# sdiehl/sonic

Measured on AMD Instinct MI355X. Metric: prove() proofs/sec, higher is better.
Workload: dtype u32 limbs (Fq 12x32, Fr 8x32 Montgomery); 1 GPU; prove(): rndCircuit n=2^18, Q=2, SRS d=2^21 (d=8n >= 7n, Protocol.hs:54); n=262144, Q=2, d=2097152, process_group=none (plain single-process run), legs=headline only (the other legs: --full)

## Files before the change

sonic_amd/csrc/device.hip:

```cpp
#include <stdarg.h>
#include <string.h>
#include <memory>
#include <string>
#include <vector>
#include "internal.hpp"

namespace sonic {

static thread_local char g_err[512] = "";
void set_error(const char* fmt, ...) {
  va_list ap;
  va_start(ap, fmt);
  vsnprintf(g_err, sizeof g_err, fmt, ap);
  va_end(ap);
}

Profiler& profiler() { static Profiler p; return p; }
void Profiler::collect() {
  std::lock_guard<std::mutex> g(mu);
  for (auto& kv : recs) {
    auto& tot = totals[kv.first];
    for (auto& r : kv.second) {
      hipEventSynchronize(r.b);
      float ms = 0;
      hipEventElapsedTime(&ms, r.a, r.b);
      tot.first += ms; tot.second += 1;
      hipEventDestroy(r.a); hipEventDestroy(r.b);
    }
    kv.second.clear();
  }
}
void Profiler::reset() { collect(); std::lock_guard<std::mutex> g(mu); totals.clear(); }

static std::mutex g_init_mu;
static int g_device = -1;
static int g_device_count = -1;
static std::vector<DeviceCtx*> g_ctx;
static thread_local DeviceCtx* t_ctx = nullptr;

static int device_count_locked() {
  if (g_device_count >= 0) return g_device_count;
  setenv("GPU_MAX_HW_QUEUES", "8", 0);
  int n = 0;
  hipError_t e = hipGetDeviceCount(&n);
  if (e != hipSuccess || n <= 0) {
    (void)hipGetLastError();
    set_error("no HIP device available (%s): libsonic_hip has no CPU fallback", e == hipSuccess ? "0 devices" : hipGetErrorString(e));
    throw HipFail{SONIC_ERR_NO_DEVICE};
  }
  g_device_count = n;
  g_ctx.assign((size_t)n, nullptr);
  return n;
}
static DeviceCtx* ctx_locked(int dev) {
  if (!g_ctx[(size_t)dev]) {
    std::unique_ptr<DeviceCtx> c(new DeviceCtx());
    c->dev = dev;
    HIP_OK(hipStreamCreateWithFlags(&c->stream, hipStreamNonBlocking));
    g_ctx[(size_t)dev] = c.release();
  }
  return g_ctx[(size_t)dev];
}
int default_device_ordinal() { std::lock_guard<std::mutex> g(g_init_mu); return g_device; }
void unlink_one_shot_of(const sonic_srs* s) {
  std::lock_guard<std::mutex> g(g_init_mu);
  for (DeviceCtx* c : g_ctx) {
    if (!c) continue;
    std::lock_guard<std::mutex> g2(c->one_shot_mu);
    for (size_t i = 0; i < c->one_shot.size();) {
      if (static_cast<OneShotShell*>(c->one_shot[i])->srs == s) c->one_shot.erase(c->one_shot.begin() + (long)i);
      else i++;
    }
  }
}

DeviceScope::DeviceScope(int dev) : ctx_(nullptr), prev_ctx_(t_ctx), prev_dev_(-1) {
  if (t_ctx && (dev < 0 || t_ctx->dev == dev)) { ctx_ = t_ctx; return; }
  std::lock_guard<std::mutex> g(g_init_mu);
  const int n = device_count_locked();
  if (dev < 0) {
    if (g_device < 0) {
      const char* lr = getenv("LOCAL_RANK");
      g_device = lr ? atoi(lr) % n : 0;
      if (g_device < 0) g_device = 0;
    }
    dev = g_device;
  }
  if (dev >= n) { set_error("device %d out of range (%d device%s)", dev, n, n == 1 ? "" : "s"); throw HipFail{SONIC_ERR_INVALID_ARG}; }
  if (hipGetDevice(&prev_dev_) != hipSuccess) { (void)hipGetLastError(); prev_dev_ = -1; }
  if (prev_dev_ != dev) HIP_OK(hipSetDevice(dev));
  try { ctx_ = ctx_locked(dev); } catch (...) { if (prev_dev_ >= 0 && prev_dev_ != dev) (void)hipSetDevice(prev_dev_); throw; }
  t_ctx = ctx_;
}
DeviceScope::~DeviceScope() {
  if (ctx_ == prev_ctx_) return;
  t_ctx = prev_ctx_;
  if (prev_dev_ >= 0 && prev_dev_ != ctx_->dev) (void)hipSetDevice(prev_dev_);
}
const NttTables& device_ntt_tables(int log2n) {
  DeviceCtx& c = current_ctx();
  std::lock_guard<std::mutex> g(c.pool_mu);
  NttTables*& t = c.prover_ntt[log2n];
  if (!t) {
    std::unique_ptr<NttTables> nt(new NttTables());
    hipStream_t st = nullptr;
    HIP_OK(hipStreamCreateWithFlags(&st, hipStreamNonBlocking));
    try { nt->ensure(st, log2n); HIP_OK(hipStreamSynchronize(st)); } catch (...) { (void)hipStreamDestroy(st); throw; }
    (void)hipStreamDestroy(st);
    t = nt.release();
  }
  return *t;
}
DeviceCtx& current_ctx() {
  if (!t_ctx) { set_error("internal: no device scope on this thread"); throw HipFail{SONIC_ERR_HIP}; }
  return *t_ctx;
}

CallLease::CallLease() : c_(nullptr), owner_(&current_ctx()) {
  {
    std::lock_guard<std::mutex> g(owner_->pool_mu);
    if (!owner_->pool.empty()) { c_ = owner_->pool.back(); owner_->pool.pop_back(); }
  }
  if (!c_) {
    std::unique_ptr<CallCtx> c(new CallCtx());
    HIP_OK(hipStreamCreateWithFlags(&c->st, hipStreamNonBlocking));
    c_ = c.release();
  }
}
CallLease::~CallLease() {
  (void)hipStreamSynchronize(c_->st);
  std::lock_guard<std::mutex> g(owner_->pool_mu);
  owner_->pool.push_back(c_);
}

}

using namespace sonic;

extern "C" {

int sonic_init(int device_ordinal) {
  API_HOST_BEGIN
  {
    std::lock_guard<std::mutex> g(g_init_mu);
    const int n = device_count_locked();
    if (device_ordinal >= n) { set_error("device %d out of range (%d device%s)", device_ordinal, n, n == 1 ? "" : "s"); return SONIC_ERR_INVALID_ARG; }
    if (g_device < 0 && device_ordinal >= 0) g_device = device_ordinal;
  }
  int dev;
  { DeviceScope scope(-1); dev = scope.ctx().dev; }
  HIP_OK(hipSetDevice(dev));
  API_END
}

int sonic_device_count(int* out) {
  if (!out) return SONIC_ERR_INVALID_ARG;
  try { std::lock_guard<std::mutex> g(g_init_mu); *out = device_count_locked(); } catch (const HipFail& f) { *out = 0; return f.code; }
  return SONIC_OK;
}

int sonic_hip_versions(int* build, int* runtime) {
  if (build) *build = HIP_VERSION;
  if (runtime) { int v = 0; if (hipRuntimeGetVersion(&v) != hipSuccess) v = 0; *runtime = v; }
  return SONIC_OK;
}

int sonic_last_error(char* buf, size_t cap) {
  if (!buf || cap == 0) return SONIC_ERR_INVALID_ARG;
  strncpy(buf, g_err, cap - 1);
  buf[cap - 1] = 0;
  return SONIC_OK;
}

int sonic_device_sync(void) { API_BEGIN HIP_OK(hipStreamSynchronize(default_stream())); HIP_OK(hipDeviceSynchronize()); API_END }

int sonic_abi_version(void) { return SONIC_ABI_VERSION; }

static int device_of_pointer(const void* p) {
  hipPointerAttribute_t a;
  if (p && hipPointerGetAttributes(&a, p) == hipSuccess) return a.device;
  (void)hipGetLastError();
  return -1;
}
int sonic_dev_alloc(size_t bytes, void** out) { return sonic_dev_alloc_on(-1, bytes, out); }
int sonic_dev_alloc_on(int device, size_t bytes, void** out) { API_BEGIN_ON(device) if (!out) return SONIC_ERR_INVALID_ARG; HIP_OK(hipMalloc(out, bytes ? bytes : 16)); API_END }
int sonic_dev_free(void* p) { API_BEGIN_ON(device_of_pointer(p)) HIP_OK(hipFree(p)); API_END }
int sonic_dev_upload(void* dst, const void* src, size_t bytes) { API_BEGIN_ON(device_of_pointer(dst)) HIP_OK(hipMemcpy(dst, src, bytes, hipMemcpyHostToDevice)); API_END }
int sonic_dev_download(void* dst, const void* src, size_t bytes) { API_BEGIN_ON(device_of_pointer(src)) HIP_OK(hipMemcpy(dst, src, bytes, hipMemcpyDeviceToHost)); API_END }

int sonic_profile_enable(int on) { profiler().on = on != 0; return SONIC_OK; }
int sonic_profile_reset(void) { profiler().reset(); return SONIC_OK; }
int sonic_profile_get(const char* kernel, double* total_ms, int64_t* launches) {
  if (!kernel) return SONIC_ERR_INVALID_ARG;
  profiler().collect();
  std::lock_guard<std::mutex> g(profiler().mu);
  auto it = profiler().totals.find(kernel);
  if (total_ms) *total_ms = it == profiler().totals.end() ? 0.0 : it->second.first;
  if (launches) *launches = it == profiler().totals.end() ? 0 : it->second.second;
  return SONIC_OK;
}
int sonic_profile_names(char* buf, size_t cap) {
  if (!buf || cap == 0) return SONIC_ERR_INVALID_ARG;
  profiler().collect();
  std::lock_guard<std::mutex> g(profiler().mu);
  std::string s;
  for (auto& kv : profiler().totals) { s += kv.first; s += "\n"; }
  strncpy(buf, s.c_str(), cap - 1);
  buf[cap - 1] = 0;
  return SONIC_OK;
}

}
```

sonic_amd/csrc/internal.hpp:

```cpp
#pragma once
#include <atomic>
#include <exception>
#include "common.hpp"
#include "g1.hpp"
#include "msm.hpp"

struct sonic_srs;
struct sonic_prover;

namespace sonic {

struct NttTables;

struct CallCtx;
struct DeviceCtx {
  int dev = -1;
  hipStream_t stream = nullptr;
  std::mutex call_mu;
  std::mutex pool_mu;
  std::vector<CallCtx*> pool;
  std::vector<void*> lanes;
  NttTables* ntt = nullptr;
  DevBuf mul_a, mul_b, mul_flags;
  std::atomic<int> sort_staged{-1};
  std::atomic<int> ntt_big{-1};
  std::map<int, NttTables*> prover_ntt;
  std::mutex one_shot_mu;
  std::vector<void*> one_shot;
};
const NttTables& device_ntt_tables(int log2n);
void drop_one_shot_of(const sonic_srs* s);
struct OneShotShell { const sonic_srs* srs; sonic_prover* p; };
void unlink_one_shot_of(const sonic_srs* s);
class DeviceScope {
 public:
  explicit DeviceScope(int dev = -1);
  ~DeviceScope();
  DeviceScope(const DeviceScope&) = delete;
  DeviceScope& operator=(const DeviceScope&) = delete;
  DeviceCtx& ctx() const { return *ctx_; }
 private:
  DeviceCtx* ctx_;
  DeviceCtx* prev_ctx_;
  int prev_dev_;
};
DeviceCtx& current_ctx();
int default_device_ordinal();
inline hipStream_t default_stream() { return current_ctx().stream; }
inline std::mutex& call_mutex() { return current_ctx().call_mu; }
struct CallCtx { hipStream_t st = nullptr; MsmWorkspace ws; };
class CallLease {
 public:
  CallLease();
  ~CallLease();
  CallLease(const CallLease&) = delete;
  CallLease& operator=(const CallLease&) = delete;
  hipStream_t st() const { return c_->st; }
  MsmWorkspace& ws() const { return c_->ws; }
 private:
  CallCtx* c_;
  DeviceCtx* owner_;
};

#define API_BEGIN_ON(dev) try { ::sonic::DeviceScope _scope(dev);
#define API_BEGIN API_BEGIN_ON(-1)
#define API_HOST_BEGIN try {
#define API_CATCH                                                               \
  } catch (const ::sonic::HipFail& f) { return f.code; }                        \
  catch (const std::exception& e) { ::sonic::set_error("%s", e.what()); return SONIC_ERR_HIP; }
#define API_END API_CATCH return SONIC_OK;

int64_t srs_d(const sonic_srs* s);
int srs_cached_id(const sonic_srs* s, int (*make)(const sonic_srs*, uint8_t*), uint8_t out[32]);

void fr_to_mont_enqueue(hipStream_t st, Fr* d, long n, int* d_err);
void fr_from_mont_enqueue(hipStream_t st, Fr* d, long n);
void fr_check_enqueue(hipStream_t st, const Fr* d, long n, int* d_err);
void points_from_bytes_enqueue(hipStream_t st, const uint8_t* d_in96, PointArrayMut out, long n, int* d_err, long inf_ok);
void points_subgroup_check_enqueue(hipStream_t st, PointArray in, long n, int* d_err);
void points_to_bytes_enqueue(hipStream_t st, PointArray in, uint8_t* d_out96, long n);
int read_flags(hipStream_t st, DevBuf& flags);
void msm_blocking(hipStream_t st, MsmWorkspace& ws, const MsmPlan& pl, PointArray d_pts, const Fr* d_sc, long n, bool mont,
                  uint8_t* out96, uint8_t* out_partial192);
struct G2Affine;
void srs_generate_g2(hipStream_t st, long d, const Fr& x_std, const Fr& alpha_std, G2Affine* h0, G2Affine* h1);
void g2_points_to_bytes_enqueue(hipStream_t st, const G2Affine* in, uint8_t* d_out, long n);
void g2_points_from_bytes_enqueue(hipStream_t st, const uint8_t* d_in, G2Affine* out, long n, int* d_err);

void g1_decompress_enqueue(hipStream_t st, const uint8_t* d_in48, PointArrayMut out, uint8_t* d_bytes96, uint8_t* d_flags, long n, bool check_subgroup);
void g2_decompress_enqueue(hipStream_t st, const uint8_t* d_in96, G2Affine* out, uint8_t* d_bytes192, uint8_t* d_flags, long n, bool check_subgroup);
void g1_compress_enqueue(hipStream_t st, PointArray in, uint8_t* d_out48, long n);
void g2_compress_enqueue(hipStream_t st, const G2Affine* in, uint8_t* d_out96, long n);
void g1_validate_enqueue(hipStream_t st, const uint8_t* d_in96, G1Affine* out, uint8_t* d_flags, long n);

struct NttTables {
  int log2n = 0;
  DevBuf fwd, inv;
  DevBuf ninv;
  void ensure(hipStream_t st, int log2n);
};
void ntt_forward_enqueue(hipStream_t st, const NttTables& tw, Fr* d, int log2n);
void ntt_inverse_enqueue(hipStream_t st, const NttTables& tw, Fr* d, int log2n);
void ntt_inverse_of_product_enqueue(hipStream_t st, const NttTables& tw, Fr* d, const Fr* other, int log2n);
void fr_pointwise_mul_enqueue(hipStream_t st, Fr* a, const Fr* b, long n);
void fr_scale_enqueue(hipStream_t st, Fr* a, long n, const Fr* d_s);
void fr_bitrev_permute_enqueue(hipStream_t st, Fr* d, int log2n);

void poly_scale_powers_enqueue(hipStream_t st, const Fr* in, Fr* out, long n, long e0, const Fr* d_x, const Fr* d_xinv);
void poly_prefix_sum_enqueue(hipStream_t st, Fr* d, long n, DevBuf& tmp);
void poly_quotient_enqueue(hipStream_t st, const Fr* prefix, Fr* q, long n, long lo, const Fr* d_z, const Fr* d_zinv);

}
```

sonic_amd/csrc/prove.hip:

```cpp
#include "prover.hpp"
#include "witness_tree.hpp"

namespace sonic {

constexpr long PROVE_TWO_LEVEL_MAX_TERMS = 1L << 21;
static bool prove_two_level(const MsmPlan& pl, int k, bool last, long nmax) {
  if (last || k <= 1 || pl.NB < (1 << 18)) return false;
  const char* e = getenv("SONIC_PROVE_TWO_LEVEL");
  if (e && (e[0] == '0' || e[0] == '1') && !e[1]) return e[0] == '1';
  return nmax <= PROVE_TWO_LEVEL_MAX_TERMS;
}
static int prove_segment(const MsmPlan& pl, int k, bool last, bool two_level) {
  const bool big = pl.NB >= (1 << 18);
  if (last) return big ? 16 : 4;
  if (k <= 1) return big ? 8 : 4;
  if (!big) return 16;
  const char* e = getenv("SONIC_PROVE_SEGMENT");
  const int v = e ? atoi(e) : 0;
  return v >= 8 && v <= 1024 ? v : (two_level ? 32 : 64);
}

MsmJob commit_job(hipStream_t st, const sonic_srs* srs, const Fr* poly, long lo, long len, long maxm, MsmSlot* slot, int* d_flags) {
  const long d = srs->d, shift = d - maxm;
  long i0 = -d - shift - lo, i1 = d - shift - lo + 1;
  if (i0 < 0) i0 = 0;
  if (i1 > len) i1 = len;
  if (i1 < i0) i1 = i0;
  flag_nonzero_enqueue(st, poly, i0, d_flags, FLAG_SRS_INDEX);
  flag_nonzero_enqueue(st, poly + i1, len - i1, d_flags, FLAG_SRS_INDEX);
  const long ih = -shift - lo;
  if (ih >= i0 && ih < i1) flag_nonzero_enqueue(st, poly + ih, 1, d_flags, FLAG_SRS_INDEX);
  return MsmJob{srs->basis(1) + (lo + i0 + shift + d), poly + i0, i1 - i0, slot};
}

void run_jobs(hipStream_t st, const sonic_srs* srs, MsmWorkspace& ws, const MsmJob* jobs, int k, bool last, bool exposed) {
  if (k <= 0) return;
  long nmax = 0;
  for (int j = 0; j < k; j++) nmax = std::max(nmax, jobs[j].n);
  MsmPlan pl = srs_msm_plan(srs, nmax);
  const bool tree = last || exposed || pl.NB <= (1 << 17);
  if (k > 1 && msm_can_batch(pl)) {
    pl.two_level = prove_two_level(pl, k, last, nmax);
    msm_plan_set_segment(pl, prove_segment(pl, k, last, pl.two_level));
    pl.tree = tree;
    msm_enqueue_batch(st, ws, pl, jobs, k, true);
    return;
  }
  for (int j = 0; j < k; j++) {
    MsmPlan p1 = srs_msm_plan(srs, jobs[j].n);
    msm_plan_set_segment(p1, prove_segment(p1, 1, false, false));
    p1.tree = tree;
    msm_enqueue_batch(st, ws, p1, &jobs[j], 1, true);
  }
}

static void eval_prefix_enqueue(hipStream_t st, Scratch& sc, const Fr* poly, long lo, long len, const Fr* zpair, Fr* d_fz) {
  sc.reserve(len);
  sc.scan.ensure(sizeof(Fr) * (len / 1024 + 2));
  poly_scale_powers_enqueue(st, poly, sc.D.as<Fr>(), len, lo, zpair, zpair + 1);
  poly_prefix_sum_enqueue(st, sc.D.as<Fr>(), len, sc.scan);
  HIP_OK(hipMemcpyAsync(d_fz, sc.D.as<Fr>() + (len - 1), sizeof(Fr), hipMemcpyDeviceToDevice, st));
}

static MsmJob quotient_job(hipStream_t st, const sonic_srs* srs, const Fr* q, long lo, long len, MsmSlot* slot, int* d_flags) {
  const long d = srs->d, qn = len - 1;
  long i0 = -d - lo, i1 = d - lo + 1;
  if (i0 < 0) i0 = 0;
  if (i1 > qn) i1 = qn;
  if (i1 < i0) i1 = i0;
  flag_nonzero_enqueue(st, q, i0, d_flags, FLAG_SRS_INDEX);
  flag_nonzero_enqueue(st, q + i1, qn - i1, d_flags, FLAG_SRS_INDEX);
  return MsmJob{srs->basis(0) + (lo + i0 + d), q + i0, i1 - i0, slot};
}

MsmJob open_job(hipStream_t st, const sonic_srs* srs, Scratch& sc, const Fr* poly, long lo, long len,
                       const Fr* zpair, Fr* d_fz, MsmSlot* slot, int* d_flags) {
  sc.reserve(len);
  eval_prefix_enqueue(st, sc, poly, lo, len, zpair, d_fz ? d_fz : sc.fz_discard.as<Fr>());
  poly_quotient_enqueue(st, sc.D.as<Fr>(), sc.q.as<Fr>(), len, lo, zpair, zpair + 1);
  return quotient_job(st, srs, sc.q.as<Fr>(), lo, len, slot, d_flags);
}

MsmJob open_job_at_zero(hipStream_t st, const sonic_srs* srs, const Fr* poly, long len, Fr* d_fz, MsmSlot* slot, int* d_flags) {
  const long d = srs->d;
  HIP_OK(hipMemcpyAsync(d_fz, poly, sizeof(Fr), hipMemcpyDeviceToDevice, st));
  const long qn = len - 1;
  long i1 = d + 1;
  if (i1 > qn) i1 = qn;
  flag_nonzero_enqueue(st, poly + 1 + i1, qn - i1, d_flags, FLAG_SRS_INDEX);
  return MsmJob{srs->basis(0) + d, poly + 1, i1, slot};
}

struct PendingOpen { const Fr* poly; long lo, len; const Fr* zp; Fr* fz; MsmSlot* slot; long slot_index; Scratch* sc; };
static void open_batch_set(OpenBatch& b, int i, Scratch& sc, const Fr* poly, long len, const Fr* zp, Fr* fz) {
  sc.reserve(len);
  sc.scan.ensure(sizeof(Fr) * (len / 1024 + 2));
  b.poly[i] = poly; b.D[i] = sc.D.as<Fr>(); b.q[i] = sc.q.as<Fr>(); b.tiles[i] = sc.scan.as<Fr>();
  b.zpair[i] = zp; b.fz[i] = fz ? fz : sc.fz_discard.as<Fr>();
}
static void open_jobs_batched(hipStream_t st, const sonic_srs* srs, const PendingOpen* ops, int k, int* d_flags, MsmJob* jobs_out) {
  for (int at = 0; at < k;) {
    int e = at;
    OpenBatch b;
    memset(&b, 0, sizeof b);
    while (e < k && e - at < OPEN_BATCH_MAX && ops[e].lo == ops[at].lo && ops[e].len == ops[at].len) {
      open_batch_set(b, e - at, *ops[e].sc, ops[e].poly, ops[e].len, ops[e].zp, ops[e].fz);
      e++;
    }
    b.k = e - at;
    const long lo = ops[at].lo, len = ops[at].len;
    open_batch_enqueue(st, b, lo, len);
    for (int i = at; i < e; i++) jobs_out[i] = quotient_job(st, srs, ops[i].sc->q.as<Fr>(), lo, len, ops[i].slot, d_flags);
    at = e;
  }
}

bool bytes_are_zero(const uint8_t* p, size_t n) { for (size_t i = 0; i < n; i++) if (p[i]) return false; return true; }

}

int upload_fr_mont(hipStream_t st, DevBuf& dst, const uint8_t* src, long count, int* d_flags) {
  dst.ensure(sizeof(Fr) * (count > 0 ? count : 1));
  if (count > 0) {
    HIP_OK(hipMemcpyAsync(dst.p, src, 32 * count, hipMemcpyHostToDevice, st));
    fr_to_mont_enqueue(st, dst.as<Fr>(), count, d_flags);
  }
  return 0;
}

int flags_to_status(int f, const char* who) {
  if (f & FLAG_BAD_ENCODING) { set_error("%s: non-canonical field element in input", who); return SONIC_ERR_BAD_ENCODING; }
  if (f & FLAG_SRS_INDEX) { set_error("%s: a non-zero coefficient needs an SRS element outside [-d, d] or the omitted g^alpha (index -1)", who); return SONIC_ERR_SRS_INDEX; }
  return SONIC_OK;
}

void prover_hand_over(sonic_prover_t* p, const CircuitView& c) {
  p->circuit_has_runs = circuit_runs_hint(c, RUN_TILE);
  p->pend.view = c;
  if (c.csr) csr_layout(c, p->pend.layout);
  p->pend.set = true;
}

static void upload_i32(hipStream_t st, DevBuf& dst, const std::vector<int32_t>& src) {
  dst.ensure(sizeof(int32_t) * (src.empty() ? 1 : src.size()));
  if (!src.empty()) HIP_OK(hipMemcpyAsync(dst.p, src.data(), sizeof(int32_t) * src.size(), hipMemcpyHostToDevice, st));
}
static void prover_upload_circuit(sonic_prover_t* p, hipStream_t st, int* d_flags) {
  const CircuitView& c = p->pend.view;
  const long n = p->n, Q = p->Q;
  if (c.csr) {
    const CsrLayout& L = p->pend.layout;
    sonic_prover::CsrBufs& b = p->sp;
    upload_i32(st, b.row_ptr, L.row_ptr); upload_i32(st, b.col, L.col);
    upload_i32(st, b.col_ptr, L.col_ptr); upload_i32(st, b.row, L.row);
    upload_i32(st, b.chunk_row, L.chunk_row); upload_i32(st, b.chunk_begin, L.chunk_begin); upload_i32(st, b.row_chunk, L.row_chunk);
    upload_fr_mont(st, b.val, c.val, L.nnz, d_flags);
    upload_fr_mont(st, b.cval, L.cval.data(), L.nnz, d_flags);
    b.nnz = L.nnz;
    b.nchunks = (long)L.chunk_row.size();
    b.partial.ensure(sizeof(Fr) * (b.nchunks > 0 ? b.nchunks : 1));
    b.h_row_ptr = L.row_ptr;
  } else {
    upload_fr_mont(st, p->wL, c.wL, Q * n, d_flags);
    upload_fr_mont(st, p->wR, c.wR, Q * n, d_flags);
    upload_fr_mont(st, p->wO, c.wO, Q * n, d_flags);
  }
  upload_fr_mont(st, p->cs, c.cs, Q, d_flags);
  p->csr = c.csr;
  p->pend.set = false;
}

static int prover_load_circuit(sonic_prover* p, const CircuitView& c) {
  hipStream_t st = p->st;
  prover_hand_over(p, c);
  HIP_OK(hipMemsetAsync(p->flags.p, 0, 4, st));
  prover_upload_circuit(p, st, p->flags.as<int>());
  int f = read_flags(st, p->flags);
  p->pend = sonic_prover::PendingCircuit();
  if (f) return flags_to_status(f, c.csr ? "sonic_prover_new_csr" : "sonic_prover_new");
  return SONIC_OK;
}

static void s_of_y_of(sonic_prover* p, hipStream_t st, const Fr* ypow, Fr* out) {
  if (p->csr) s_of_y_csc_enqueue(st, p->sp.col_ptr.as<int32_t>(), p->sp.row.as<int32_t>(), p->sp.cval.as<Fr>(), ypow, p->n, p->Q, out);
  else s_of_y_enqueue(st, p->wL.as<Fr>(), p->wR.as<Fr>(), p->wO.as<Fr>(), ypow, p->n, p->Q, out);
}
static void s_of_u_of(sonic_prover* p, hipStream_t st, const Fr* upow, Fr* out) {
  sonic_prover::CsrBufs& b = p->sp;
  if (p->csr) s_of_u_csr_enqueue(st, b.row_ptr.as<int32_t>(), b.col.as<int32_t>(), b.val.as<Fr>(), b.chunk_row.as<int32_t>(), b.chunk_begin.as<int32_t>(),
                                 b.nchunks, b.row_chunk.as<int32_t>(), upow, p->n, p->Q, out, b.partial.as<Fr>());
  else s_of_u_enqueue(st, p->wL.as<Fr>(), p->wR.as<Fr>(), p->wO.as<Fr>(), upow, p->n, p->Q, out, p->tmp);
}

extern "C" {

size_t sonic_proof_size(int64_t Q) { return ProofLayout{Q}.proof_bytes(); }

static int prover_new_entry(const char* who, const sonic_srs_t* srs, const CircuitView& c, sonic_prover_t** out) {
  API_BEGIN_ON(srs_device(srs))
  if (!srs || !c.cs || !out) { set_error("%s: bad argument (need n >= 1, Q >= 1)", who); return SONIC_ERR_INVALID_ARG; }
  int rc = prover_admits(who, srs, c);
  if (rc) return rc;
  return prover_new_impl(srs, c, out);
  API_END
}
int sonic_prover_new(const sonic_srs_t* srs, int64_t n, int64_t Q, const uint8_t* wL, const uint8_t* wR, const uint8_t* wO,
                     const uint8_t* cs, sonic_prover_t** out) {
  return prover_new_entry("sonic_prover_new", srs, dense_view(n, Q, wL, wR, wO, cs), out);
}
int sonic_prover_new_csr(const sonic_srs_t* srs, int64_t n, int64_t Q, const int64_t* row_ptr, const int64_t* col, const uint8_t* val,
                         const uint8_t* cs, sonic_prover_t** out) {
  return prover_new_entry("sonic_prover_new_csr", srs, csr_view(n, Q, row_ptr, col, val, cs), out);
}

}

int prover_admits(const char* who, const sonic_srs* srs, const CircuitView& c) {
  if (circuit_args_ok(c) && srs->d < 7 * c.n) {
    set_error("Parameter d is not large enough: %ld should be greater than %ld", (long)srs->d, (long)(7 * c.n));
    return SONIC_ERR_D_TOO_SMALL;
  }
  return circuit_validate(who, c);
}

int prover_new_impl(const sonic_srs_t* srs, const CircuitView& c, sonic_prover_t** out) {
  const long n = c.n, Q = c.Q;
  const ProofLayout L{Q};
  for (long q = 0; c.csr && q < Q; q++) {
    Fr k; memcpy(k.l, c.cs + 32 * q, 32);
    if (!fp_is_canonical(k)) { set_error("sonic_prover_new_csr: non-canonical constant cs[%ld]", q); return SONIC_ERR_BAD_ENCODING; }
  }
  std::unique_ptr<sonic_prover> p(new sonic_prover());
  p->srs = srs; p->n = n; p->Q = Q;
  p->device = srs_device(srs);
  {
    const MsmPlan probe = srs_msm_plan(srs, 3 * n);
    p->small_plan = msm_can_batch(probe) && probe.NB <= (1 << 17);
  }
  auto mkstream = [](hipStream_t* s) { HIP_OK(hipStreamCreateWithFlags(s, hipStreamNonBlocking)); };
  mkstream(&p->st);
  mkstream(&p->ts);
  hipStream_t st = p->st;
  p->flags.alloc(8);
  int rc_c = prover_load_circuit(p.get(), c);
  if (rc_c) return rc_c;
  const long tlen = 7 * n + 9;
  int lg = 0;
  while ((1L << lg) < tlen) lg++;
  p->log2m = lg;
  p->ntt = &device_ntt_tables(lg);
  const long M = 1L << lg;
  p->fa.alloc(sizeof(Fr) * M); p->fb.alloc(sizeof(Fr) * M);
  p->r1.alloc(sizeof(Fr) * (3 * n + 5));
  p->sy0.alloc(sizeof(Fr) * (3 * n + 1));
  p->syj.resize(Q);
  for (auto& b : p->syj) b.alloc(sizeof(Fr) * (3 * n + 1));
  p->su.alloc(sizeof(Fr) * (2 * n + Q + 1));
  p->pw.alloc(sizeof(Fr) * (3 * n + Q + 2));
  p->kpow.alloc(sizeof(Fr) * Q);
  p->S.alloc(sizeof(Fr) * L.transcript_len()); p->PAIRS.alloc(sizeof(Fr) * 2 * L.n_pairs());
  p->slots.alloc(sizeof(MsmSlot) * L.slots_total());
  p->use_graph = getenv("SONIC_PROVE_GRAPH") && atoi(getenv("SONIC_PROVE_GRAPH")) != 0;
  HIP_OK(hipHostMalloc((void**)&p->h_tr, 32 * L.transcript_len(), hipHostMallocDefault));
  HIP_OK(hipHostMalloc((void**)&p->h_pairs, sizeof(Fr) * 2 * L.n_pairs(), hipHostMallocDefault));
  HIP_OK(hipHostMalloc((void**)&p->h_slots, sizeof(MsmSlot) * L.slots_total(), hipHostMallocDefault));
  HIP_OK(hipHostMalloc((void**)&p->h_fr, 32 * L.F(), hipHostMallocDefault));
  HIP_OK(hipHostMalloc((void**)&p->h_flags, 8, hipHostMallocDefault));
  HIP_OK(hipHostMalloc((void**)&p->h_root, 32, hipHostMallocDefault));
  p->h_flags[0] = p->h_flags[1] = 0;
  p->frout.alloc(sizeof(Fr) * L.F());
  p->frstd.alloc(sizeof(Fr) * L.F());
  HIP_OK(hipMemsetAsync(p->frout.p, 0, sizeof(Fr) * L.F(), st));
  HIP_OK(hipMemsetAsync(p->slots.p, 0, sizeof(MsmSlot) * L.slots_total(), st));
  memset(p->h_slots, 0, sizeof(MsmSlot) * L.slots_total());
  auto mkev = [](hipEvent_t* e) { HIP_OK(hipEventCreateWithFlags(e, hipEventDisableTiming)); };
  mkev(&p->ev_r1); mkev(&p->ev_sy0); mkev(&p->ev_t); mkev(&p->ev_su);
  p->ev_syj.resize(Q, nullptr);
  for (auto& e : p->ev_syj) mkev(&e);
  if (p->small_plan) {
    const char* le = getenv("SONIC_FUSED_LANES");
    p->n_lanes = std::min(std::max(le ? atoi(le) : N_LANES, 1), N_LANES);
  }
  for (int i = 0; i < p->n_lanes; i++) {
    Lane& l = p->lanes[i];
    mkstream(&l.st);
    mkev(&l.done);
    mkev(&l.prep);
  }
  if (p->small_plan) {
    for (int c = 0; c < (L.K() > MSM_MAX_JOBS ? 2 : 1); c++) {
      mkstream(&p->chain[c].st);
      mkev(&p->chain[c].done);
    }
  }
  HIP_OK(hipStreamSynchronize(st));
  *out = p.release();
  return SONIC_OK;
}

extern "C" {

int sonic_prover_set_assignment(sonic_prover_t* p, const uint8_t* aL, const uint8_t* aR, const uint8_t* aO) {
  API_BEGIN_ON(p ? p->device : -1)
  if (!p || !aL || !aR || !aO) return SONIC_ERR_INVALID_ARG;
  std::lock_guard<std::mutex> g(p->mu);
  if (p->in_flight) { set_error("sonic_prover_set_assignment: a submitted proof is still reading the current assignment (collect it first)"); return SONIC_ERR_INVALID_ARG; }
  hipStream_t st = p->st;
  HIP_OK(hipMemsetAsync(p->flags.p, 0, 4, st));
  upload_fr_mont(st, p->aL, aL, p->n, p->flags.as<int>());
  upload_fr_mont(st, p->aR, aR, p->n, p->flags.as<int>());
  upload_fr_mont(st, p->aO, aO, p->n, p->flags.as<int>());
  int f = read_flags(st, p->flags);
  if (f) {
    p->have_assignment = false;
    return flags_to_status(f, "sonic_prover_set_assignment");
  }
  p->have_assignment = true;
  p->assignment_changed();
  API_END
}

}

struct GroupQueue {
  sonic_prover_t* const p;
  const sonic_srs* const srs;
  const ProofLayout L;
  int* const flags; MsmSlot* const slots; Fr* const frout;
  const SlotShare* const sh;
  Lane* cur = nullptr;
  std::vector<PendingOpen> pend;
  std::vector<std::function<void()>> after_flush;
  std::vector<std::function<void()>> deferred_small;
  enum Side { BESIDE_GROUP, BEHIND_CHAIN };

  explicit GroupQueue(sonic_prover_t* p_)
      : p(p_), srs(p_->srs), L{p_->Q}, flags(p_->flags.as<int>()), slots(p_->slots.as<MsmSlot>()), frout(p_->frout.as<Fr>()),
        sh(p_->share_world > 1 ? p_->share.row(p_->share_rank) : nullptr) {
    p->next_lane = 0;
    p->slot_ran.assign((size_t)L.slots_total(), 0);
    p->fr_valid.assign((size_t)L.F(), 0);
  }
  bool on(int ph) const { return ((p->phases >> ph) & 1u) != 0; }
  bool own(long slot) const { return !sh || sh[slot].hi > sh[slot].lo; }
  bool first_piece(long slot) const { return !sh || (sh[slot].hi > sh[slot].lo && sh[slot].lo == 0); }
  void push(MsmJob job, long slot) {
    if (sh) {
      long t0, t1;
      share_term_range(sh[slot], job.n, &t0, &t1);
      job.points = job.points + t0; job.scalars += t0; job.n = t1 - t0;
      if (job.n <= 0) return;
    }
    p->slot_ran[(size_t)slot] = 1;
    cur->jobs[cur->njobs++] = job;
  }
  void issue_opens() {
    if (pend.empty()) return;
    MsmJob oj[MSM_MAX_JOBS];
    open_jobs_batched(cur->st, srs, pend.data(), (int)pend.size(), flags, oj);
    for (size_t i = 0; i < pend.size(); i++) push(oj[i], pend[i].slot_index);
    pend.clear();
  }
  void flush(bool last = false) {
    if (!cur) return;
    issue_opens();
    if (p->fused) p->fused_jobs.insert(p->fused_jobs.end(), cur->jobs, cur->jobs + cur->njobs);
    else run_jobs(cur->st, srs, cur->ws, cur->jobs, cur->njobs, last, p->share_world >= 4);
    cur->njobs = 0;
    if (p->fused) deferred_small.insert(deferred_small.end(), after_flush.begin(), after_flush.end());
    else for (auto& f : after_flush) f();
    after_flush.clear();
  }
  void begin_group(hipEvent_t e) {
    flush();
    cur = &p->pick(e);
    cur->njobs = 0;
  }
  void begin_t_group(Lane& lane_t) {
    if (on(PH_T)) HIP_OK(hipStreamWaitEvent(lane_t.st, p->ev_t, 0));
    cur = &lane_t; cur->njobs = 0;
  }
  void make_room() { if (cur->njobs + (int)pend.size() == MSM_MAX_JOBS) flush(); }
  void commit(int ph, const Fr* poly, long lo, long len, long maxm, long slot) {
    if (!on(ph) || !own(slot)) return;
    make_room();
    push(commit_job(cur->st, srs, poly, lo, len, maxm, &slots[slot], flags), slot);
  }
  void commit_runs(int ph, const Fr* poly, long lo, long len, long maxm, long j) {
    const long slot = L.S(j), Q = L.Q;
    if (!on(ph) || !own(slot)) return;
    make_room();
    MsmJob job = commit_job(cur->st, srs, poly, lo, len, maxm, &slots[slot], flags);
    const long ntiles = job.n / RUN_TILE;
    if (ntiles > 0) {
      if ((long)p->runs.size() < Q) p->runs.resize((size_t)Q);
      sonic_prover::RunBufs& rb = p->runs[(size_t)j];
      if (!rb.masked_ev) HIP_OK(hipEventCreateWithFlags(&rb.masked_ev, hipEventDisableTiming));
      rb.masked.ensure(sizeof(Fr) * job.n); rb.val.ensure(sizeof(Fr) * ntiles); rb.uniform.ensure(4 * ntiles);
      rb.scal.ensure(sizeof(Fr) * 2 * ntiles); rb.pts.ensure(sizeof(G1Affine) * 2 * ntiles);
      run_tiles_enqueue(cur->st, job.scalars, job.n, rb.masked.as<Fr>(), rb.val.as<Fr>(), rb.uniform.as<uint32_t>());
      HIP_OK(hipEventRecord(rb.masked_ev, cur->st));
      const long first = (long)((job.points.p - srs->basis(1).p) / (long)job.points.stride);
      sonic_prover::RunBufs* rbp = &rb;
      side([this, rbp, first, ntiles, j] {
        hipStream_t ms = p->st;
        HIP_OK(hipStreamWaitEvent(ms, rbp->masked_ev, 0));
        run_terms_enqueue(ms, rbp->val.as<Fr>(), rbp->uniform.as<uint32_t>(), ntiles, srs->prefix() + first, first, rbp->scal.as<Fr>(), rbp->pts.as<G1Affine>());
        msm_enqueue(ms, p->runs_ws, msm_plan(2 * ntiles), PointArray::packed(rbp->pts.as<G1Affine>()), rbp->scal.as<Fr>(), 2 * ntiles, true, &slots[L.S_extra(j)]);
      }, BEHIND_CHAIN);
      job.scalars = rb.masked.as<Fr>();
      p->slot_ran[(size_t)L.S_extra(j)] = 1;
    }
    push(job, slot);
  }
  void commit_sym(int ph, const Fr* su, long lo, long len, long n) {
    if (!on(ph) || !own(L.C())) return;
    const long d = srs->d;
    make_room();
    MsmJob job = commit_job(cur->st, srs, su, lo, len, d, &slots[L.C()], flags);
    job.points = srs->sym() + 1; job.scalars = su + (n + 1); job.n = n; job.table_stride = d + 1;
    push(job, L.C());
    p->slot_ran[(size_t)L.C_extra()] = 1;
    side([this, su, d, n] { msm_enqueue(p->st, p->runs_ws, msm_plan(L.Q), srs->basis(1) + (d + n + 1), su + (2 * n + 1), L.Q, true, &slots[L.C_extra()]); }, BEHIND_CHAIN);
  }
  void open(int ph, const Fr* poly, long lo, long len, const Fr* zp, long fr, long slot) {
    if (!on(ph) || !own(slot)) return;
    make_room();
    Scratch& sc = p->fused ? p->fused_scratch() : cur->sc[cur->njobs + (int)pend.size()];
    pend.push_back(PendingOpen{poly, lo, len, zp, fr >= 0 ? &frout[fr] : nullptr, &slots[slot], slot, &sc});
    if (fr >= 0 && first_piece(slot)) p->fr_valid[(size_t)fr] = 1;
  }
  void side(std::function<void()> fn, Side when) {
    if (when == BEHIND_CHAIN ? !p->fused : cur->njobs == 0) fn();
    else (when == BEHIND_CHAIN ? deferred_small : after_flush).push_back(std::move(fn));
  }
  void run_chains() {
    if (!p->fused || p->fused_jobs.empty()) return;
    for (int i = 0; i < p->n_lanes; i++) HIP_OK(hipEventRecord(p->lanes[i].prep, p->lanes[i].st));
    const int total = (int)p->fused_jobs.size();
    const int nchunks = (total + MSM_MAX_JOBS - 1) / MSM_MAX_JOBS, per = (total + nchunks - 1) / nchunks;
    for (int c = 0, at = 0; c < nchunks; c++, at += per) {
      Lane& cl = p->chain[c & 1];
      if (c < 2) for (int i = 0; i < p->n_lanes; i++) HIP_OK(hipStreamWaitEvent(cl.st, p->lanes[i].prep, 0));
      const int k = std::min(per, total - at);
      const MsmJob* jobs = &p->fused_jobs[(size_t)at];
      long nmax = 0;
      for (int j = 0; j < k; j++) nmax = std::max(nmax, jobs[j].n);
      MsmPlan pl = srs_msm_plan(srs, nmax);
      pl.tree = true;
      pl.accum_block = 128;
      msm_enqueue_batch(cl.st, cl.ws, pl, jobs, k, true);
    }
    p->fused_jobs.clear();
  }
  void drain_deferred() {
    for (auto& f : deferred_small) f();
    deferred_small.clear();
  }
  void join() {
    hipStream_t ms = p->st;
    for (int i = 0; i < p->n_lanes; i++) { Lane& l = p->lanes[i]; HIP_OK(hipEventRecord(l.done, l.st)); HIP_OK(hipStreamWaitEvent(ms, l.done, 0)); }
    if (p->fused) for (auto& l : p->chain) if (l.st) { HIP_OK(hipEventRecord(l.done, l.st)); HIP_OK(hipStreamWaitEvent(ms, l.done, 0)); }
  }
};

struct ProofPass {
  const long n, Q, d;
  const long r_lo, r_len, s_lo, s_len, t_lo, t_len, u_lo, u_len;
  const Fr* const PR;
  bool need_g0, need_T, need_su, need_j_any = false;
  std::vector<uint8_t> need_j;
  long last_j = -1;
  int last_group;
  bool g0_queued = false;
  const Fr* pair(long i) const { return PR + 2 * i; }
  ProofPass(sonic_prover_t* p, const GroupQueue& q)
      : n(p->n), Q(p->Q), d(p->srs->d), r_lo(-2 * n - 4), r_len(3 * n + 5), s_lo(-n), s_len(3 * n + 1), t_lo(-4 * n - 8), t_len(7 * n + 9),
        u_lo(-n), u_len(2 * n + Q + 1), PR(p->PAIRS.as<Fr>()), need_j((size_t)Q, 0) {
    const ProofLayout& L = q.L;
    need_su = q.own(L.C()) || q.own(L.Qv());
    for (long j = 0; j < Q; j++) {
      need_j[(size_t)j] = q.own(L.S(j)) || q.own(L.W(j)) || q.own(L.Wp(j));
      need_j_any = need_j_any || need_j[(size_t)j];
      if (need_j[(size_t)j]) last_j = j;
      need_su = need_su || q.own(L.Qj(j));
    }
    need_g0 = q.own(L.R) || q.own(L.Wa) || q.own(L.Wb);
    need_T = q.own(L.T) || q.own(L.Wt);
    last_group = need_T ? 3 : need_su ? 2 : need_j_any ? 1 : 0;
  }
};

static void enqueue_group0(sonic_prover_t* p, GroupQueue& q, ProofPass& w) {
  if (!w.need_g0 || w.g0_queued) return;
  w.g0_queued = true;
  const ProofLayout& L = q.L;
  const Fr* r1 = p->r1.as<Fr>();
  q.begin_group(p->ev_r1);
  q.commit(PH_R, r1, w.r_lo, w.r_len, w.n, L.R);
  q.open(PH_OPEN, r1, w.r_lo, w.r_len, w.pair(L.pZ), L.a, L.Wa);
  q.open(PH_OPEN, r1, w.r_lo, w.r_len, w.pair(L.pYZ), L.b, L.Wb);
  q.flush(w.last_group == 0);
}

static void enqueue_polynomials(sonic_prover_t* p, GroupQueue& q, ProofPass& w) {
  const ProofLayout& L = q.L;
  const long n = w.n, Q = w.Q;
  hipStream_t ms = p->st;
  int* flags = q.flags;
  Fr *r1 = p->r1.as<Fr>(), *sy = p->sy0.as<Fr>(), *pw = p->pw.as<Fr>(), *fa = p->fa.as<Fr>(), *fb = p->fb.as<Fr>();
  auto ready = [&](hipEvent_t e) { HIP_OK(hipEventRecord(e, ms)); };
  if (p->pend_asg[0]) {
    upload_fr_mont(ms, p->aL, p->pend_asg[0], n, flags + 1);
    upload_fr_mont(ms, p->aR, p->pend_asg[1], n, flags + 1);
    upload_fr_mont(ms, p->aO, p->pend_asg[2], n, flags + 1);
    p->pend_asg[0] = nullptr;
    p->assignment_changed();
  }
  if (p->pend_wit.set) {
    for (DevBuf* a : {&p->aL, &p->aR, &p->aO}) a->ensure(sizeof(Fr) * (size_t)n);
    if (p->pend_wit.ready) HIP_OK(hipStreamWaitEvent(ms, p->pend_wit.ready, 0));
    witness_load_enqueue(p, ms, p->pend_wit.v, 1, p->aL.as<Fr>(), p->aR.as<Fr>(), p->aO.as<Fr>(), n, flags + 1);
    p->pend_wit.set = false;
    p->assignment_changed();
  }
  if (p->pend_cs) {
    upload_fr_mont(ms, p->cs, p->pend_cs, Q, flags + 1);
    p->pend_cs = nullptr;
  }
  if ((w.need_g0 || w.need_T) && q.on(PH_R)) build_r1_enqueue(ms, p->aL.as<Fr>(), p->aR.as<Fr>(), p->aO.as<Fr>(), p->S.as<Fr>(), n, r1);
  ready(p->ev_r1);
  if (p->pend.set) {
    enqueue_group0(p, q, w);
    prover_upload_circuit(p, ms, flags + 1);
  }
  if (w.need_T && q.on(PH_T)) {
    poly_scale_powers_enqueue(ms, nullptr, pw, 2 * n + Q + 1, -n, w.pair(L.pY), w.pair(L.pY) + 1);
    s_of_y_of(p, ms, pw, sy);
    HIP_OK(hipMemcpyAsync(p->kpow.p, pw + (2 * n + 1), sizeof(Fr) * Q, hipMemcpyDeviceToDevice, ms));
  }
  ready(p->ev_sy0);
  if (w.need_T && q.on(PH_T)) {
    hipStream_t ts = p->ts;
    const long M = 1L << p->log2m;
    HIP_OK(hipStreamWaitEvent(ts, p->ev_sy0, 0));
    t_operands_enqueue(ts, r1, w.r_len, w.r_lo, sy, w.s_lo - w.r_lo, w.s_len, w.pair(L.pY), fa, fb, M);
    ntt_forward_enqueue(ts, *p->ntt, fa, p->log2m);
    ntt_forward_enqueue(ts, *p->ntt, fb, p->log2m);
    ntt_inverse_of_product_enqueue(ts, *p->ntt, fa, fb, p->log2m);
    sub_k_of_y_enqueue(ts, fa + (0 - w.t_lo), p->cs.as<Fr>(), p->kpow.as<Fr>(), Q, flags, 0);
    HIP_OK(hipEventRecord(p->ev_t, ts));
  }
  for (long j = 0; j < Q; j++) {
    if (w.need_j[(size_t)j] && q.on(PH_HSCS)) {
      poly_scale_powers_enqueue(ms, nullptr, pw, 2 * n + Q + 1, -n, w.pair(L.pYj(j)), w.pair(L.pYj(j)) + 1);
      if (!p->prepared || q.own(L.W(j)) || q.own(L.Wp(j))) s_of_y_of(p, ms, pw, p->syj[j].as<Fr>());
      if (p->prepared && q.own(L.S(j))) s_diag_part_enqueue(ms, pw, n, Q, p->diag[j].as<Fr>(), p->yq[j].as<Fr>());
    }
    ready(p->ev_syj[j]);
  }
  if (w.need_su && q.on(PH_HSCW)) {
    poly_scale_powers_enqueue(ms, nullptr, pw, 3 * n + 1, -n, w.pair(L.pU), w.pair(L.pU) + 1);
    s_of_u_of(p, ms, pw, p->su.as<Fr>());
  }
  ready(p->ev_su);
}

static void enqueue_t_group(sonic_prover_t* p, GroupQueue& q, const ProofPass& w, Lane& lane_t) {
  const ProofLayout& L = q.L;
  const Fr* t = p->fa.as<Fr>();
  q.begin_t_group(lane_t);
  q.commit(PH_T, t, w.t_lo, w.t_len, w.d, L.T);
  q.open(PH_OPEN, t, w.t_lo, w.t_len, w.pair(L.pZ), -1, L.Wt);
  q.flush(true);
}

static void enqueue_groups(sonic_prover_t* p, GroupQueue& q, ProofPass& w) {
  const ProofLayout& L = q.L;
  const long n = w.n, Q = w.Q, d = w.d;
  MsmSlot* slots = q.slots;
  Fr* su = p->su.as<Fr>();
  Lane& lane_t = p->t_lane(p->ev_sy0);
  if (q.on(PH_OPEN) && q.first_piece(L.Wt)) {
    OpenBatch eb;
    memset(&eb, 0, sizeof eb);
    eb.k = 1;
    open_batch_set(eb, 0, lane_t.sc[MSM_MAX_JOBS - 1], p->sy0.as<Fr>(), w.s_len, w.pair(L.pZ), &q.frout[L.s]);
    open_batch_enqueue(lane_t.st, eb, w.s_lo, w.s_len, false);
    p->fr_valid[(size_t)L.s] = 1;
  }
  enqueue_group0(p, q, w);
  for (long j = 0; j < Q; j++) {
    if (!w.need_j[(size_t)j]) continue;
    Fr* syj = p->syj[j].as<Fr>();
    q.begin_group(p->ev_syj[j]);
    if (p->prepared) q.commit(PH_HSCS, p->diag[j].as<Fr>(), n + 1, n, d, L.S(j));
    else if (p->runs_on) q.commit_runs(PH_HSCS, syj, w.s_lo, w.s_len, d, j);
    else q.commit(PH_HSCS, syj, w.s_lo, w.s_len, d, L.S(j));
    q.open(PH_HSCS, syj, w.s_lo, w.s_len, w.pair(L.pZj(j)), L.s_j(j), L.W(j));
    q.open(PH_HSCW, syj, w.s_lo, w.s_len, w.pair(L.pU), -1, L.Wp(j));
    q.flush(w.last_group == 1 && j == w.last_j);
    if (p->prepared && q.on(PH_HSCS) && q.first_piece(L.S(j))) {
      Lane* ln = q.cur;
      p->slot_ran[(size_t)L.S_extra(j)] = 1;
      q.side([p, ln, j, Q, out = &slots[L.S_extra(j)]] {
        msm_enqueue(ln->st, ln->ws, p->cq_tab.p ? msm_plan_tables(Q, CQ_TAB_C, CQ_TAB_W, Q) : msm_plan(Q),
                    PointArray::packed(p->cq_tab.p ? p->cq_tab.as<G1Affine>() : p->cq.as<G1Affine>()), p->yq[j].as<Fr>(), Q, true, out);
      }, GroupQueue::BESIDE_GROUP);
    }
  }
  if (w.need_su) {
    q.begin_group(p->ev_su);
    if (p->sym_on) q.commit_sym(PH_HSCW, su, w.u_lo, w.u_len, n);
    else q.commit(PH_HSCW, su, w.u_lo, w.u_len, d, L.C());
    for (long j = 0; j < Q; j++) q.open(PH_HSCW, su, w.u_lo, w.u_len, w.pair(L.pYj(j)), L.sp_j(j), L.Qj(j));
    q.open(PH_QV, su, w.u_lo, w.u_len, w.pair(L.pV), -1, L.Qv());
  }
  q.flush(w.last_group == 2 && q.sh != nullptr);
  if (w.need_T) enqueue_t_group(p, q, w, lane_t);
  q.run_chains();
  q.drain_deferred();
}

static void enqueue_proof(sonic_prover_t* p) {
  const ProofLayout L{p->Q};
  hipStream_t st = p->st;
  int* flags = p->flags.as<int>();
  HIP_OK(hipMemsetAsync(flags, 0, 8, st));
  Fr* S = p->S.as<Fr>();
  HIP_OK(hipMemcpyAsync(S, p->h_tr, 32 * L.transcript_len(), hipMemcpyHostToDevice, st));
  fr_to_mont_enqueue(st, S, L.transcript_len(), flags);
  HIP_OK(hipMemcpyAsync(p->PAIRS.p, p->h_pairs, sizeof(Fr) * 2 * L.n_pairs(), hipMemcpyHostToDevice, st));
  GroupQueue q(p);
  ProofPass w(p, q);
  enqueue_polynomials(p, q, w);
  enqueue_groups(p, q, w);
  q.join();
  Fr* frstd = p->frstd.as<Fr>();
  HIP_OK(hipMemcpyAsync(frstd, q.frout, sizeof(Fr) * L.F(), hipMemcpyDeviceToDevice, st));
  fr_from_mont_enqueue(st, frstd, L.F());
  const long KS = p->sym_on ? L.slots_total() : (p->prepared || p->runs_on) ? L.C_extra() : L.K();
  HIP_OK(hipMemcpyAsync(p->h_slots, q.slots, sizeof(MsmSlot) * KS, hipMemcpyDeviceToHost, st));
  HIP_OK(hipMemcpyAsync(p->h_fr, frstd, 32 * L.F(), hipMemcpyDeviceToHost, st));
  HIP_OK(hipMemcpyAsync(p->h_flags, flags, 8, hipMemcpyDeviceToHost, st));
}

static void decide_modes(sonic_prover_t* p) {
  {
    const char* re = getenv("SONIC_PROVE_RUNS");
    const int mode = re ? atoi(re) : -1;
    const bool size_ok = mode == 1 ? 3 * p->n + 1 >= 8 * RUN_TILE : p->n >= (1L << 16);
    p->runs_on = mode != 0 && size_ok && (mode == 1 || p->circuit_has_runs) && !p->prepared && p->share_world <= 1 && p->srs->prefix().p != nullptr;
  }
  {
    const char* se = getenv("SONIC_PROVE_SYM");
    const int mode = se ? atoi(se) : -1;
    p->sym_on = mode != 0 && (mode == 1 || p->n >= (1L << 17)) && p->share_world <= 1 && p->srs->sym().p != nullptr;
  }
  {
    const MsmPlan probe = srs_msm_plan(p->srs, 3 * p->n);
    const char* fe = getenv("SONIC_PROVE_FUSED");
    const int mode = fe ? atoi(fe) : -1;
    p->fused = mode != 0 && p->small_plan && msm_can_batch(probe) && p->share_world <= 1;
    p->fused_jobs.clear();
    p->fused_sc_next = 0;
  }
}

static void share_replan_if_needed(sonic_prover_t* p) {
  if (p->share_world <= 1 || (p->share_planned && p->share_planned_prepared == p->prepared)) return;
  const long n = p->n, Q = p->Q;
  const MsmPlan mp = srs_msm_plan(p->srs, 3 * n);
  const ShareCosts costs = ShareCosts::from_env();
  p->share = share_plan(n, Q, p->prepared, p->share_world, mp.NB, mp.W, costs);
  uint64_t h = 1469598103934665603ull;
  auto mix = [&](uint64_t v) { for (int i = 0; i < 8; i++) { h ^= (v >> (8 * i)) & 0xff; h *= 1099511628211ull; } };
  auto mixd = [&](double d) { uint64_t v; memcpy(&v, &d, 8); mix(v); };
  mix((uint64_t)n); mix((uint64_t)Q); mix(p->prepared ? 1 : 0); mix((uint64_t)p->share_world); mix((uint64_t)mp.NB); mix((uint64_t)mp.W);
  mixd(costs.per_job_buckets); mixd(costs.r1); mixd(costs.sy); mixd(costs.su); mixd(costs.tprod);
  p->share_plan_tag = (int32_t)(uint32_t)(h ^ (h >> 32));
  p->share_planned = true; p->share_planned_prepared = p->prepared;
}

static void challenge_pairs_host(sonic_prover_t* p, const uint8_t* transcript) {
  const ProofLayout L{p->Q};
  const long np = L.n_pairs();
  std::vector<Fr> v((size_t)np), pre((size_t)np);
  auto tr = [&](long k) { Fr a; memcpy(a.l, transcript + 32 * k, 32); return fp_to_mont(a); };
  v[L.pY] = tr(L.y); v[L.pZ] = tr(L.z); v[L.pYZ] = fp_mul(v[L.pY], v[L.pZ]); v[L.pU] = tr(L.u()); v[L.pV] = tr(L.v());
  for (long j = 0; j < L.Q; j++) { v[L.pYj(j)] = tr(L.y_j(j)); v[L.pZj(j)] = tr(L.z_j(j)); }
  Fr acc = Fr::one();
  for (long i = 0; i < np; i++) { pre[i] = acc; acc = fp_mul(acc, v[i].is_zero() ? Fr::one() : v[i]); }
  Fr inv = fp_inv(acc);
  for (long i = np - 1; i >= 0; i--) {
    p->h_pairs[2 * i] = v[i];
    if (v[i].is_zero()) { p->h_pairs[2 * i + 1] = v[i]; continue; }
    p->h_pairs[2 * i + 1] = fp_mul(inv, pre[i]);
    inv = fp_mul(inv, v[i]);
  }
}

static int prove_enqueue(sonic_prover_t* p, const uint8_t* transcript) {
  API_BEGIN_ON(p->device)
  p->t_begin = std::chrono::steady_clock::now();
  const ProofLayout L{p->Q};
  hipStream_t st = p->st;
  for (long k = L.n_blinders; k < L.transcript_len(); k++)
    if (bytes_are_zero(transcript + 32 * k, 32)) { set_error("prove: transcript element %ld is zero: Laurent evaluation at 0 divides by zero", k); return SONIC_ERR_INEXACT_DIVISION; }
  if (p->share_world > 1 && p->phases != PH_ALL) { set_error("prove: a shared proof runs with a caller-supplied transcript only"); return SONIC_ERR_INVALID_ARG; }
  decide_modes(p);
  share_replan_if_needed(p);
  memcpy(p->h_tr, transcript, 32 * L.transcript_len());
  challenge_pairs_host(p, transcript);
  const bool pending = p->pend.set || p->pend_asg[0] != nullptr || p->pend_wit.set || p->pend_cs != nullptr;
  const bool want_graph = p->use_graph && p->proofs_done >= 1 && !profiler().on && p->phases == PH_ALL && !pending;
  const bool replay = want_graph && p->graph != nullptr;
  const bool capturing = want_graph && !replay && !p->graph_tried;
  struct CaptureGuard {
    hipStream_t st; bool active = false;
    ~CaptureGuard() { if (active) { hipGraph_t g = nullptr; (void)hipStreamEndCapture(st, &g); if (g) (void)hipGraphDestroy(g); } }
  } capture{st};
  if (capturing) { p->graph_tried = true; HIP_OK(hipStreamBeginCapture(st, hipStreamCaptureModeRelaxed)); capture.active = true; }
  if (!replay) enqueue_proof(p);
  if (capturing) {
    hipGraph_t g = nullptr;
    capture.active = false;
    HIP_OK(hipStreamEndCapture(st, &g));
    hipError_t ge = hipGraphInstantiate(&p->graph, g, nullptr, nullptr, 0);
    (void)hipGraphDestroy(g);
    if (ge != hipSuccess) { p->graph = nullptr; set_error("prove: hipGraphInstantiate failed: %s", hipGetErrorString(ge)); return SONIC_ERR_HIP; }
  }
  if (replay || capturing) HIP_OK(hipGraphLaunch(p->graph, st));
  p->t_enq = std::chrono::steady_clock::now();
  API_END
}

namespace {
struct ShareHeader { uint32_t magic, version; int32_t rank, world; int64_t Q; int32_t flags, plan_tag; };
constexpr uint32_t SHARE_VERSION = 2;
constexpr uint32_t SHARE_MAGIC = 0x48534e53u;
G1XYZZ g1_sum(const G1XYZZ& a, const G1XYZZ& b) { return g1_add(a, b); }
}
extern "C" size_t sonic_proof_share_size(int64_t Q) {
  const size_t K = (size_t)ProofLayout{Q}.K(), F = (size_t)ProofLayout{Q}.F();
  return sizeof(ShareHeader) + K * 8 + K * 192 + F * 32 + F * 4;
}

static bool await_proof(sonic_prover_t* p, bool share) {
  HIP_OK(hipStreamSynchronize(p->st));
  p->proofs_done++;
  if (!getenv("SONIC_DEBUG_TIMING")) return false;
  char who[32] = "prove";
  if (share) snprintf(who, sizeof who, "share %d/%d", p->share_rank, p->share_world);
  fprintf(stderr, "[sonic] %s: enqueue %.3f ms, then waited %.3f ms for the device\n", who,
          std::chrono::duration<double, std::milli>(p->t_enq - p->t_begin).count(),
          std::chrono::duration<double, std::milli>(std::chrono::steady_clock::now() - p->t_enq).count());
  return true;
}

static int prove_finish_share(sonic_prover_t* p, uint8_t* out_share) {
  API_BEGIN_ON(p->device)
  const long Q = p->Q;
  const ProofLayout L{Q};
  const int K = (int)L.K(), F = (int)L.F();
  await_proof(p, true);
  const MsmSlot* hs = p->h_slots;
  memset(out_share, 0, sonic_proof_share_size(Q));
  ShareHeader h{SHARE_MAGIC, SHARE_VERSION, p->share_rank, p->share_world > 1 ? p->share_world : 1, Q, *p->h_flags, p->share_world > 1 ? p->share_plan_tag : 0};
  memcpy(out_share, &h, sizeof h);
  uint8_t* o = out_share + sizeof h;
  for (int i = 0; i < K; i++) {
    SlotShare s; s.lo = 0; s.hi = SHARE_ONE;
    if (p->share_world > 1) s = p->share.row(p->share_rank)[i];
    memcpy(o, &s.lo, 4); memcpy(o + 4, &s.hi, 4); o += 8;
  }
  std::vector<G1XYZZ> sums((size_t)L.slots_total());
  for (long i = 0; i < L.slots_total(); i++) sums[(size_t)i] = p->slot_ran[(size_t)i] ? msm_finish_host(hs[i]) : G1XYZZ::inf();
  fold_side_slots(L, p->prepared || p->runs_on, p->sym_on, sums.data(), sums.data() + K, g1_sum);
  memcpy(o, sums.data(), 192 * (size_t)K);
  o += 192 * (size_t)K;
  for (int i = 0; i < F; i++, o += 32) if (p->fr_valid[(size_t)i]) memcpy(o, p->h_fr + 32 * i, 32);
  for (int i = 0; i < F; i++, o += 4) { const int32_t v = p->fr_valid[(size_t)i]; memcpy(o, &v, 4); }
  API_END
}

extern "C" int sonic_proof_from_shares(int64_t Q, int world, const uint8_t* shares, const uint8_t* transcript, uint8_t* out_proof) {
  try {
  if (Q < 1 || world < 1 || !shares || !transcript || !out_proof) return SONIC_ERR_INVALID_ARG;
  const int K = (int)ProofLayout{Q}.K(), F = (int)ProofLayout{Q}.F();
  const size_t sz = sonic_proof_share_size(Q);
  std::vector<const uint8_t*> by_rank((size_t)world, nullptr);
  int flags = 0;
  int32_t tag0 = 0;
  for (int r = 0; r < world; r++) {
    ShareHeader h;
    memcpy(&h, shares + sz * r, sizeof h);
    if (r == 0) tag0 = h.plan_tag;
    if (h.magic == SHARE_MAGIC && h.version == SHARE_VERSION && h.plan_tag != tag0) {
      set_error("sonic_proof_from_shares: the ranks planned the proof with different parameters (share %d: tag %08x, share 0: %08x) -- their SRS handles "
                "run different MSM plans (window tables built on one GPU and not on another?) or their SONIC_SHARE_COST_* environments differ", r, (unsigned)h.plan_tag, (unsigned)tag0);
      return SONIC_ERR_INVALID_ARG;
    }
    if (h.magic != SHARE_MAGIC || h.version != SHARE_VERSION || h.Q != Q || h.world != world || h.rank < 0 || h.rank >= world || by_rank[(size_t)h.rank]) {
      set_error("sonic_proof_from_shares: share %d is not one of %d distinct shares of a Q = %ld proof", r, world, (long)Q); return SONIC_ERR_INVALID_ARG; }
    by_rank[(size_t)h.rank] = shares + sz * r;
    flags |= h.flags;
  }
  if (flags) return flags_to_status(flags, "prove");
  std::vector<G1XYZZ> sums((size_t)K, G1XYZZ::inf());
  for (int i = 0; i < K; i++) {
    std::vector<std::pair<uint32_t, uint32_t>> pieces;
    for (int r = 0; r < world; r++) {
      const uint8_t* b = by_rank[(size_t)r] + sizeof(ShareHeader);
      uint32_t lo, hi;
      memcpy(&lo, b + 8 * i, 4); memcpy(&hi, b + 8 * i + 4, 4);
      if (hi <= lo) continue;
      pieces.push_back({lo, hi});
      G1XYZZ part;
      memcpy(&part, b + 8 * K + 192 * (size_t)i, 192);
      sums[(size_t)i] = g1_add(sums[(size_t)i], part);
    }
    std::sort(pieces.begin(), pieces.end());
    uint32_t at = 0;
    for (auto& pc : pieces) { if (pc.first != at) break; at = pc.second; }
    if (at != SHARE_ONE) { set_error("sonic_proof_from_shares: the pieces of MSM %d do not cover its terms exactly once", i); return SONIC_ERR_INVALID_ARG; }
  }
  std::vector<uint8_t> pts(96 * (size_t)K), frs(32 * (size_t)F);
  g1_canonical_bytes_host_batch(sums.data(), K, pts.data());
  for (int i = 0; i < F; i++) {
    bool got = false;
    for (int r = 0; r < world && !got; r++) {
      const uint8_t* b = by_rank[(size_t)r] + sizeof(ShareHeader) + 8 * (size_t)K + 192 * (size_t)K;
      int32_t v; memcpy(&v, b + 32 * (size_t)F + 4 * (size_t)i, 4);
      if (v) { memcpy(&frs[32 * (size_t)i], b + 32 * (size_t)i, 32); got = true; }
    }
    if (!got) { set_error("sonic_proof_from_shares: no share reports evaluation %d", i); return SONIC_ERR_INVALID_ARG; }
  }
  proof_layout(Q, pts.data(), frs.data(), transcript, out_proof);
  } catch (const std::exception& e) { set_error("%s", e.what()); return SONIC_ERR_HIP; }
  return SONIC_OK;
}

static bool slots_folded(const MsmSlot* hs, long K) {
  for (long i = 0; i < K; i++) if (hs[i].W > 1 && hs[i].pad1 == 0) return false;
  return true;
}
static void finish_slots_host(const MsmSlot* hs, long K, G1XYZZ* out, int max_threads) {
  long two_level = 0;
  for (long i = 0; i < K; i++) two_level += hs[i].pad1 == 3;
  const int nt = !slots_folded(hs, K) ? (int)std::min<long>(K, max_threads) : (two_level >= 8 ? std::min(4, max_threads) : 1);
  ThreadGroup th;
  for (int w = 1; w < nt; w++) th.emplace_back([=] { for (long i = w; i < K; i += nt) out[i] = msm_finish_host(hs[i]); });
  for (long i = 0; i < K; i += nt) out[i] = msm_finish_host(hs[i]);
}

static int prove_finish(sonic_prover_t* p, uint8_t* out_proof) {
  API_BEGIN_ON(p->device)
  const long Q = p->Q;
  const ProofLayout L{Q};
  const int K = (int)L.K();
  const uint8_t* transcript = p->h_tr;
  const bool timing = await_proof(p, false);
  const MsmSlot* hs = p->h_slots;
  const uint8_t* hfr_p = p->h_fr;
  const int hflags = *p->h_flags;
  if (p->h_flags[1]) { p->have_assignment = false; return flags_to_status(p->h_flags[1], "prove (circuit / assignment handed over with the call)"); }
  if (hflags) return flags_to_status(hflags, "prove");
  std::vector<uint8_t> pts(96 * (size_t)K);
  {
    auto t0 = std::chrono::steady_clock::now();
    std::vector<G1XYZZ> sums((size_t)K);
    const bool has_extra = p->prepared || p->runs_on;
    std::vector<G1XYZZ> side((size_t)(Q + 1), G1XYZZ::inf());
    const MsmSlot* hx = hs + L.S_extra(0);
    ThreadGroup th;
    if (p->sym_on) th.emplace_back([&] { side[(size_t)Q] = msm_finish_host(hs[L.C_extra()]); });
    if (has_extra && !slots_folded(hx, Q)) th.emplace_back([&] { finish_slots_host(hx, Q, side.data(), 8); });
    else if (has_extra) finish_slots_host(hx, Q, side.data(), 1);
    finish_slots_host(hs, K, sums.data(), 16);
    th.join();
    fold_side_slots(L, has_extra, p->sym_on, sums.data(), side.data(), g1_sum);
    g1_canonical_bytes_host_batch(sums.data(), K, pts.data());
    if (timing) fprintf(stderr, "[sonic] host tails of %d MSMs: %.3f ms\n", K, std::chrono::duration<double, std::milli>(std::chrono::steady_clock::now() - t0).count());
  }
  proof_layout(Q, pts.data(), hfr_p, transcript, out_proof);
  API_END
}

extern "C" {

static int whole_proof_only(sonic_prover_t* p, const char* who) {
  if (p->share_world > 1) { set_error("%s: the handle runs one rank's share of a proof (sonic_prover_set_share): use collect_share / prove_share", who); return SONIC_ERR_INVALID_ARG; }
  return SONIC_OK;
}

static int fs_flight_refused(sonic_prover_t* p, const char* who) {
  if (p->fs_flight) { set_error("%s: the proof in flight was submitted with sonic_prover_submit_fs: collect it with sonic_prover_collect_fs", who); return SONIC_ERR_INVALID_ARG; }
  return SONIC_OK;
}

static int prove_args_ok(sonic_prover_t* p, const char* who) {
  if (!p->have_assignment) { set_error("%s: no assignment set", who); return SONIC_ERR_INVALID_ARG; }
  if (p->in_flight) { set_error("%s: a submitted proof has not been collected yet", who); return SONIC_ERR_INVALID_ARG; }
  return SONIC_OK;
}

static int prove_run(sonic_prover_t* p, const uint8_t* transcript, int (*finish)(sonic_prover_t*, uint8_t*), uint8_t* out) {
  int rc = prove_enqueue(p, transcript);
  if (rc) { if (p->st) (void)hipStreamSynchronize(p->st); return rc; }
  return finish ? finish(p, out) : SONIC_OK;
}

int sonic_prover_prove(sonic_prover_t* p, const uint8_t* transcript, uint8_t* out_proof) {
  if (!p || !transcript || !out_proof) return SONIC_ERR_INVALID_ARG;
  std::lock_guard<std::mutex> g(p->mu);
  int rc = prove_args_ok(p, "sonic_prover_prove");
  if (!rc) rc = whole_proof_only(p, "sonic_prover_prove");
  if (!rc) rc = prove_run(p, transcript, prove_finish, out_proof);
  return rc;
}

int prove_with_statement(sonic_prover_t* p, const uint8_t* aL, const uint8_t* aR, const uint8_t* aO, const uint8_t* cs, const uint8_t* transcript,
                         uint8_t* out_proof) {
  std::lock_guard<std::mutex> g(p->mu);
  if (p->in_flight) { set_error("prove: a submitted proof has not been collected yet"); return SONIC_ERR_INVALID_ARG; }
  int rc = whole_proof_only(p, "prove");
  if (rc) return rc;
  if (!aL && !p->have_assignment) { set_error("prove: no assignment set"); return SONIC_ERR_INVALID_ARG; }
  if (aL) { p->pend_asg[1] = aR; p->pend_asg[2] = aO; p->pend_asg[0] = aL; }
  p->pend_cs = cs;
  rc = prove_run(p, transcript, prove_finish, out_proof);
  p->pend_asg[0] = nullptr;
  p->pend_cs = nullptr;
  if (aL) p->have_assignment = rc == SONIC_OK;
  return rc;
}

int prove_with_witness(sonic_prover_t* p, const WitnessView& w, hipEvent_t ready, const uint8_t* cs, const uint8_t* transcript, uint8_t* out_proof) {
  std::lock_guard<std::mutex> g(p->mu);
  if (p->in_flight) { set_error("prove: a submitted proof has not been collected yet"); return SONIC_ERR_INVALID_ARG; }
  int rc = whole_proof_only(p, "prove");
  if (rc) return rc;
  p->pend_wit.v = w; p->pend_wit.ready = ready; p->pend_wit.set = true;
  p->pend_cs = cs;
  rc = prove_run(p, transcript, prove_finish, out_proof);
  p->pend_wit.set = false;
  p->pend_cs = nullptr;
  p->have_assignment = rc == SONIC_OK;
  return rc;
}

int sonic_prover_submit(sonic_prover_t* p, const uint8_t* transcript) {
  if (!p || !transcript) return SONIC_ERR_INVALID_ARG;
  std::lock_guard<std::mutex> g(p->mu);
  int rc = prove_args_ok(p, "sonic_prover_submit");
  if (!rc) rc = prove_run(p, transcript, nullptr, nullptr);
  if (!rc) p->in_flight = true;
  return rc;
}

int sonic_prover_collect(sonic_prover_t* p, uint8_t* out_proof) {
  if (!p || !out_proof) return SONIC_ERR_INVALID_ARG;
  std::lock_guard<std::mutex> g(p->mu);
  if (!p->in_flight) { set_error("sonic_prover_collect: nothing was submitted"); return SONIC_ERR_INVALID_ARG; }
  if (fs_flight_refused(p, "sonic_prover_collect")) return SONIC_ERR_INVALID_ARG;
  if (whole_proof_only(p, "sonic_prover_collect")) return SONIC_ERR_INVALID_ARG;
  p->in_flight = false;
  return prove_finish(p, out_proof);
}

int sonic_prover_set_share(sonic_prover_t* p, int rank, int world) {
  API_BEGIN_ON(p ? p->device : -1)
  if (!p || (world > 1 && (rank < 0 || rank >= world))) return SONIC_ERR_INVALID_ARG;
  std::lock_guard<std::mutex> g(p->mu);
  if (p->in_flight) { set_error("sonic_prover_set_share: a submitted proof has not been collected yet"); return SONIC_ERR_INVALID_ARG; }
  if (p->graph) { (void)hipGraphExecDestroy(p->graph); p->graph = nullptr; }
  p->graph_tried = false;
  p->share_rank = world > 1 ? rank : 0;
  p->share_world = world > 1 ? world : 0;
  p->share_planned = false;
  HIP_OK(hipMemsetAsync(p->slots.p, 0, sizeof(MsmSlot) * ProofLayout{p->Q}.C_extra(), p->st));
  HIP_OK(hipMemsetAsync(p->frout.p, 0, sizeof(Fr) * ProofLayout{p->Q}.F(), p->st));
  HIP_OK(hipStreamSynchronize(p->st));
  API_END
}

int sonic_prover_collect_share(sonic_prover_t* p, uint8_t* out_share) {
  if (!p || !out_share) return SONIC_ERR_INVALID_ARG;
  std::lock_guard<std::mutex> g(p->mu);
  if (!p->in_flight) { set_error("sonic_prover_collect_share: nothing was submitted"); return SONIC_ERR_INVALID_ARG; }
  if (fs_flight_refused(p, "sonic_prover_collect_share")) return SONIC_ERR_INVALID_ARG;
  p->in_flight = false;
  return prove_finish_share(p, out_share);
}

int sonic_prover_prove_share(sonic_prover_t* p, const uint8_t* transcript, uint8_t* out_share) {
  if (!p || !transcript || !out_share) return SONIC_ERR_INVALID_ARG;
  std::lock_guard<std::mutex> g(p->mu);
  int rc = prove_args_ok(p, "sonic_prover_prove_share");
  if (!rc) rc = prove_run(p, transcript, prove_finish_share, out_share);
  return rc;
}

int sonic_prove_share_plan(int64_t n, int64_t Q, int prepared, int world, int rank, int64_t nb, int w, uint32_t* out_lo_hi, double* out_cost) {
  if (n < 1 || Q < 1 || world < 1 || rank < 0 || rank >= world || !out_lo_hi) return SONIC_ERR_INVALID_ARG;
  const SharePlan pl = share_plan(n, Q, prepared != 0, world, nb > 0 ? nb : (1L << 19), w > 0 ? w : 13, ShareCosts::from_env());
  for (int i = 0; i < pl.K; i++) { out_lo_hi[2 * i] = pl.row(rank)[i].lo; out_lo_hi[2 * i + 1] = pl.row(rank)[i].hi; }
  if (out_cost) *out_cost = pl.cost[(size_t)rank];
  return SONIC_OK;
}

int sonic_fs_circuit_digest(int64_t n, int64_t Q, const uint8_t* wL, const uint8_t* wR, const uint8_t* wO, const uint8_t* cs, uint8_t out[32]) {
  return circuit_digest_checked("sonic_fs_circuit_digest", dense_view(n, Q, wL, wR, wO, cs), out);
}

int sonic_fs_challenges_v2(int64_t n, int64_t Q, int64_t d, const uint8_t circuit_digest[32], const uint8_t srs_id[32], const uint8_t* proof, uint8_t* out) {
  if (n < 1 || Q < 1 || d < 1 || !circuit_digest || !srs_id || !proof || !out) return SONIC_ERR_INVALID_ARG;
  fs_challenges_of_proof(n, Q, d, circuit_digest, srs_id, proof, out);
  return SONIC_OK;
}
int sonic_fs_challenges(int64_t, int64_t, int64_t, const uint8_t*, const uint8_t*, uint8_t*) {
  set_error("sonic_fs_challenges is retired (the transcript binds the SRS since round 4): use sonic_fs_challenges_v2, which takes the srs id");
  return SONIC_ERR_INVALID_ARG;
}

static void witness_digest_v1_ensure(sonic_prover_t* p) {
  if (p->have_witness_digest) return;
  const long n = p->n;
  DevBuf tmp(sizeof(Fr) * 3 * n);
  Fr* t3 = tmp.as<Fr>();
  HIP_OK(hipMemcpyAsync(t3, p->aL.p, sizeof(Fr) * n, hipMemcpyDeviceToDevice, p->st));
  HIP_OK(hipMemcpyAsync(t3 + n, p->aR.p, sizeof(Fr) * n, hipMemcpyDeviceToDevice, p->st));
  HIP_OK(hipMemcpyAsync(t3 + 2 * n, p->aO.p, sizeof(Fr) * n, hipMemcpyDeviceToDevice, p->st));
  fr_from_mont_enqueue(p->st, t3, 3 * n);
  std::vector<uint8_t> host(96 * (size_t)n);
  HIP_OK(hipMemcpyAsync(host.data(), t3, host.size(), hipMemcpyDeviceToHost, p->st));
  HIP_OK(hipStreamSynchronize(p->st));
  Sha256 h;
  h.update("sonic-hip/witness/v1", 20);
  h.update(host.data(), host.size());
  h.finish(p->witness_digest);
  p->have_witness_digest = true;
}

static void witness_digest_v2_enqueue(sonic_prover_t* p) {
  if (p->have_witness_digest_v2) return;
  const uint32_t* root = witness_tree_enqueue(p->st, p->aL.as<Fr>(), p->aR.as<Fr>(), p->aO.as<Fr>(), p->n, p->wtree);
  HIP_OK(hipMemcpyAsync(p->h_root, root, 32, hipMemcpyDeviceToHost, p->st));
}
static void witness_digest_v2_finish(sonic_prover_t* p) {
  if (p->have_witness_digest_v2) return;
  uint8_t root[32];
  wt_digest_bytes(p->h_root, root);
  fs_witness_digest_v2(p->n, root, p->witness_digest_v2);
  p->have_witness_digest_v2 = true;
}
static void witness_digest_v2_ensure(sonic_prover_t* p) {
  if (p->have_witness_digest_v2) return;
  witness_digest_v2_enqueue(p);
  HIP_OK(hipStreamSynchronize(p->st));
  witness_digest_v2_finish(p);
}

static int prove_fs_walk(sonic_prover_t* p, const uint8_t circuit_digest[32], const uint8_t blinder_seed[32], const uint8_t witness_digest[32], uint8_t* out_proof,
                         uint8_t* out_transcript) {
  int rc;
  const long n = p->n, Q = p->Q, d = p->srs->d;
  const ProofLayout L{Q};
  std::vector<uint8_t> tr(32 * (size_t)L.transcript_len(), 0), pf(sonic_proof_size(Q));
  uint8_t srs_id[32];
  if ((rc = sonic_fs_srs_id(p->srs, srs_id))) return rc;
  for (long k = 0; k < L.n_blinders; k++) fs_blinder(blinder_seed, circuit_digest, srs_id, witness_digest, (uint32_t)k, &tr[32 * k]);
  for (long k = L.n_blinders; k < L.transcript_len(); k++) tr[32 * k] = 1;
  FsTranscript t;
  t.init(n, Q, d, circuit_digest, srs_id);
  auto pass = [&](int ph) {
    p->phases = 1u << ph;
    int r = prove_run(p, tr.data(), prove_finish, pf.data());
    p->phases = PH_ALL;
    return r;
  };
  const uint8_t* R = pf.data(), * T = R + 96, * open = R + 192, * hscS = R + 576, * hscW = hscS + Q * 224, * Cc = hscW + Q * 224 + 96;
  if ((rc = pass(PH_R))) return rc;
  t.absorb("R", R, 96);
  t.challenge("y", 0, &tr[32 * L.y]);
  if ((rc = pass(PH_T))) return rc;
  t.absorb("T", T, 96);
  t.challenge("z", 0, &tr[32 * L.z]);
  if ((rc = pass(PH_OPEN))) return rc;
  t.absorb("open", open, 384);
  for (long j = 0; j < Q; j++) { t.challenge("yj", (uint32_t)j, &tr[32 * L.y_j(j)]); t.challenge("zj", (uint32_t)j, &tr[32 * L.z_j(j)]); }
  if ((rc = pass(PH_HSCS))) return rc;
  t.absorb("hscS", hscS, (size_t)Q * 224);
  t.challenge("u", 0, &tr[32 * L.u()]);
  if ((rc = pass(PH_HSCW))) return rc;
  {
    std::string w(reinterpret_cast<const char*>(Cc), 96);
    w.append(reinterpret_cast<const char*>(hscW), (size_t)Q * 224);
    t.absorb("hscW", reinterpret_cast<const uint8_t*>(w.data()), w.size());
  }
  t.challenge("v", 0, &tr[32 * L.v()]);
  if ((rc = pass(PH_QV))) return rc;
  memcpy(out_proof, pf.data(), pf.size());
  if (out_transcript) memcpy(out_transcript, tr.data(), tr.size());
  return SONIC_OK;
}

int sonic_prover_prove_fs(sonic_prover_t* p, const uint8_t circuit_digest[32], const uint8_t blinder_seed[32], uint8_t* out_proof,
                          uint8_t* out_transcript) {
  if (!p || !circuit_digest || !blinder_seed || !out_proof) return SONIC_ERR_INVALID_ARG;
  API_BEGIN_ON(p->device)
  std::lock_guard<std::mutex> g(p->mu);
  int rc = prove_args_ok(p, "sonic_prover_prove_fs");
  if (!rc) rc = whole_proof_only(p, "sonic_prover_prove_fs");
  if (rc) return rc;
  witness_digest_v1_ensure(p);
  return prove_fs_walk(p, circuit_digest, blinder_seed, p->witness_digest, out_proof, out_transcript);
  API_END
}

int sonic_prover_witness_digest_v2(sonic_prover_t* p, uint8_t out[32]) {
  API_BEGIN_ON(p ? p->device : -1)
  if (!p || !out) { set_error("sonic_prover_witness_digest_v2: bad argument"); return SONIC_ERR_INVALID_ARG; }
  std::lock_guard<std::mutex> g(p->mu);
  int rc = prove_args_ok(p, "sonic_prover_witness_digest_v2");
  if (rc) return rc;
  witness_digest_v2_ensure(p);
  memcpy(out, p->witness_digest_v2, 32);
  API_END
}

static int fs_job(sonic_prover_t* p, FsWorker& w) {
  API_BEGIN_ON(p->device)
  witness_digest_v2_ensure(p);
  return prove_fs_walk(p, w.circuit_digest, w.seed, p->witness_digest_v2, w.proof.data(), w.transcript.data());
  API_END
}
static void fs_worker_main(sonic_prover_t* p) {
  FsWorker& w = *p->fsw;
  std::unique_lock<std::mutex> lk(w.m);
  for (;;) {
    w.cv.wait(lk, [&] { return w.quit || (w.has_job && !w.done); });
    if (!(w.has_job && !w.done)) return;
    lk.unlock();
    int rc = SONIC_ERR_HIP;
    std::string err;
    try {
      rc = fs_job(p, w);
      if (rc) { char b[512]; sonic_last_error(b, sizeof b); err = b; }
    } catch (...) { rc = SONIC_ERR_HIP; err = "sonic_prover_submit_fs: the worker failed"; }
    lk.lock();
    w.rc = rc; w.err = err; w.done = true;
    w.cv.notify_all();
  }
}

int sonic_prover_submit_fs(sonic_prover_t* p, const uint8_t circuit_digest[32], const uint8_t blinder_seed[32]) {
  API_BEGIN_ON(p ? p->device : -1)
  if (!p || !circuit_digest || !blinder_seed) { set_error("sonic_prover_submit_fs: bad argument"); return SONIC_ERR_INVALID_ARG; }
  std::lock_guard<std::mutex> g(p->mu);
  int rc = prove_args_ok(p, "sonic_prover_submit_fs");
  if (!rc) rc = whole_proof_only(p, "sonic_prover_submit_fs");
  if (rc) return rc;
  if (!p->fsw) {
    p->fsw.reset(new FsWorker());
    p->fsw->th = std::thread(fs_worker_main, p);
  }
  FsWorker& w = *p->fsw;
  {
    std::lock_guard<std::mutex> gw(w.m);
    memcpy(w.circuit_digest, circuit_digest, 32); memcpy(w.seed, blinder_seed, 32);
    w.proof.assign(sonic_proof_size(p->Q), 0);
    w.transcript.assign(32 * (size_t)ProofLayout{p->Q}.transcript_len(), 0);
    w.has_job = true; w.done = false; w.rc = SONIC_OK; w.err.clear();
  }
  p->in_flight = true; p->fs_flight = true;
  w.cv.notify_all();
  API_END
}

int sonic_prover_collect_fs(sonic_prover_t* p, uint8_t* out_proof, uint8_t* out_transcript) {
  API_BEGIN_ON(p ? p->device : -1)
  if (!p || !out_proof) { set_error("sonic_prover_collect_fs: bad argument"); return SONIC_ERR_INVALID_ARG; }
  std::lock_guard<std::mutex> g(p->mu);
  if (!p->in_flight) { set_error("sonic_prover_collect_fs: nothing was submitted"); return SONIC_ERR_INVALID_ARG; }
  if (!p->fs_flight) { set_error("sonic_prover_collect_fs: the proof in flight was submitted with a transcript (sonic_prover_submit): collect it with sonic_prover_collect"); return SONIC_ERR_INVALID_ARG; }
  FsWorker& w = *p->fsw;
  std::unique_lock<std::mutex> lk(w.m);
  w.cv.wait(lk, [&] { return w.done; });
  w.has_job = false;
  p->in_flight = false; p->fs_flight = false;
  if (w.rc) { set_error("%s", w.err.c_str()); return w.rc; }
  memcpy(out_proof, w.proof.data(), w.proof.size());
  if (out_transcript) memcpy(out_transcript, w.transcript.data(), w.transcript.size());
  API_END
}

int prove_fs_with_statement(sonic_prover_t* p, const uint8_t* aL, const uint8_t* aR, const uint8_t* aO, const uint8_t* cs, const uint8_t circuit_digest[32],
                            const uint8_t blinder_seed[32], uint8_t* out_proof, uint8_t* out_transcript) {
  API_BEGIN_ON(p->device)
  std::lock_guard<std::mutex> g(p->mu);
  if (p->in_flight) { set_error("prove: a submitted proof has not been collected yet"); return SONIC_ERR_INVALID_ARG; }
  int rc = whole_proof_only(p, "prove");
  if (rc) return rc;
  if (!aL && !p->have_assignment) { set_error("prove: no assignment set"); return SONIC_ERR_INVALID_ARG; }
  hipStream_t st = p->st;
  if (aL) {
    p->have_assignment = false;
    p->assignment_changed();
    HIP_OK(hipMemsetAsync(p->flags.p, 0, 4, st));
    upload_fr_mont(st, p->aL, aL, p->n, p->flags.as<int>());
    upload_fr_mont(st, p->aR, aR, p->n, p->flags.as<int>());
    upload_fr_mont(st, p->aO, aO, p->n, p->flags.as<int>());
    witness_digest_v2_enqueue(p);
    const int f = read_flags(st, p->flags);
    if (f) return flags_to_status(f, "prove (assignment handed over with the call)");
    witness_digest_v2_finish(p);
    p->have_assignment = true;
  } else witness_digest_v2_ensure(p);
  p->pend_cs = cs;
  rc = prove_fs_walk(p, circuit_digest, blinder_seed, p->witness_digest_v2, out_proof, out_transcript);
  p->pend_cs = nullptr;
  return rc;
  API_END
}

int prove_fs_with_witness(sonic_prover_t* p, const WitnessView& w, hipEvent_t ready, const uint8_t* cs, const uint8_t circuit_digest[32],
                          const uint8_t blinder_seed[32], uint8_t* out_proof, uint8_t* out_transcript) {
  API_BEGIN_ON(p->device)
  std::lock_guard<std::mutex> g(p->mu);
  if (p->in_flight) { set_error("prove: a submitted proof has not been collected yet"); return SONIC_ERR_INVALID_ARG; }
  int rc = whole_proof_only(p, "prove");
  if (rc) return rc;
  hipStream_t st = p->st;
  p->have_assignment = false;
  p->assignment_changed();
  for (DevBuf* a : {&p->aL, &p->aR, &p->aO}) a->ensure(sizeof(Fr) * (size_t)p->n);
  if (ready) HIP_OK(hipStreamWaitEvent(st, ready, 0));
  HIP_OK(hipMemsetAsync(p->flags.p, 0, 4, st));
  witness_load_enqueue(p, st, w, 1, p->aL.as<Fr>(), p->aR.as<Fr>(), p->aO.as<Fr>(), p->n, p->flags.as<int>());
  witness_digest_v2_enqueue(p);
  const int f = read_flags(st, p->flags);
  if (f) return flags_to_status(f, "prove (assignment handed over with the call)");
  witness_digest_v2_finish(p);
  p->have_assignment = true;
  p->pend_cs = cs;
  rc = prove_fs_walk(p, circuit_digest, blinder_seed, p->witness_digest_v2, out_proof, out_transcript);
  p->pend_cs = nullptr;
  return rc;
  API_END
}

int sonic_prover_prepare(sonic_prover_t* p) {
  API_BEGIN_ON(p ? p->device : -1)
  if (!p) return SONIC_ERR_INVALID_ARG;
  std::lock_guard<std::mutex> g(p->mu);
  if (p->prepared) return SONIC_OK;
  if (p->in_flight) { set_error("sonic_prover_prepare: a submitted proof has not been collected yet"); return SONIC_ERR_INVALID_ARG; }
  if (p->graph) { (void)hipGraphExecDestroy(p->graph); p->graph = nullptr; }
  p->graph_tried = false;
  const long n = p->n, Q = p->Q, d = p->srs->d;
  int* flags = p->flags.as<int>();
  HIP_OK(hipMemsetAsync(flags, 0, 4, p->st));
  HIP_OK(hipStreamSynchronize(p->st));
  DevBuf slots(sizeof(MsmSlot) * Q);
  std::vector<DevBuf> rows(p->csr ? 0 : std::min<long>(Q, N_LANES));
  for (auto& b : rows) b.alloc(sizeof(Fr) * (3 * n + 1));
  DevBuf terms_pts, terms_scal;
  if (p->csr) {
    const std::vector<int32_t>& rp = p->sp.h_row_ptr;
    const long nnz = p->sp.nnz;
    terms_pts.alloc(sizeof(G1Affine) * (nnz > 0 ? nnz : 1));
    terms_scal.alloc(sizeof(Fr) * (nnz > 0 ? nnz : 1));
    HIP_OK(hipMemsetAsync(slots.p, 0, sizeof(MsmSlot) * Q, p->st));
    HIP_OK(hipStreamSynchronize(p->st));
    const PointArray A = p->srs->basis(1) + d;
    long at = 0;
    for (long q = 0; q < Q; q++) {
      const int32_t seg[6] = {rp[q], rp[q + 1] - rp[q], rp[Q + q], rp[Q + q + 1] - rp[Q + q], rp[2 * Q + q], rp[2 * Q + q + 1] - rp[2 * Q + q]};
      const long cnt = (long)seg[1] + seg[3] + seg[5];
      if (cnt == 0) continue;
      Lane& l = p->lane_at((int)(q % N_LANES));
      G1Affine* pts = terms_pts.as<G1Affine>() + at;
      Fr* scal = terms_scal.as<Fr>() + at;
      csr_row_terms_enqueue(l.st, p->sp.col.as<int32_t>(), p->sp.val.as<Fr>(), seg, n, A, pts, scal);
      msm_enqueue(l.st, l.ws, msm_plan(cnt), PointArray::packed(pts), scal, cnt, true, slots.as<MsmSlot>() + q);
      at += cnt;
    }
  }
  for (long q = 0; q < Q && !p->csr; q++) {
    Lane& l = p->lane_at((int)(q % N_LANES));
    Fr* row = rows[q % N_LANES].as<Fr>();
    weight_row_poly_enqueue(l.st, p->wL.as<Fr>(), p->wR.as<Fr>(), p->wO.as<Fr>(), n, q, row);
    MsmJob job = commit_job(l.st, p->srs, row, -n, 3 * n + 1, d, slots.as<MsmSlot>() + q, flags);
    run_jobs(l.st, p->srs, l.ws, &job, 1);
  }
  for (int i = 0; i < p->n_lanes; i++) HIP_OK(hipStreamSynchronize(p->lanes[i].st));
  std::vector<MsmSlot> hs(Q);
  HIP_OK(hipMemcpy(hs.data(), slots.p, sizeof(MsmSlot) * Q, hipMemcpyDeviceToHost));
  int hflags = 0;
  HIP_OK(hipMemcpy(&hflags, flags, 4, hipMemcpyDeviceToHost));
  if (hflags) return flags_to_status(hflags, "sonic_prover_prepare");
  std::vector<G1Affine> cq(Q);
  {
    std::vector<G1XYZZ> sums((size_t)Q);
    finish_slots_host(hs.data(), Q, sums.data(), 16);
    g1_batch_affine_host(sums.data(), Q, cq.data());
  }
  p->cq.alloc(sizeof(G1Affine) * Q);
  HIP_OK(hipMemcpy(p->cq.p, cq.data(), sizeof(G1Affine) * Q, hipMemcpyHostToDevice));
  if (Q <= CQ_TAB_MAX_Q) {
    std::vector<G1XYZZ> tx((size_t)CQ_TAB_W * Q);
    ThreadGroup th;
    const int nt = (int)std::min<long>(Q, 16);
    for (int t = 0; t < nt; t++)
      th.emplace_back([&, t] {
        for (long q = t; q < Q; q += nt) {
          G1XYZZ a = G1XYZZ::from_affine(cq[q]);
          tx[q] = a;
          for (int w = 1; w < CQ_TAB_W; w++) {
            for (int k = 0; k < msm_even_width(CQ_TAB_W, w - 1); k++) a = g1_dbl(a);
            tx[(size_t)w * Q + q] = a;
          }
        }
      });
    for (auto& x : th) x.join();
    std::vector<G1Affine> tab(tx.size());
    g1_batch_affine_host(tx.data(), (long)tx.size(), tab.data());
    p->cq_tab.alloc(sizeof(G1Affine) * tab.size());
    HIP_OK(hipMemcpy(p->cq_tab.p, tab.data(), sizeof(G1Affine) * tab.size(), hipMemcpyHostToDevice));
  }
  p->diag.resize(Q); p->yq.resize(Q);
  for (auto& b : p->diag) b.alloc(sizeof(Fr) * n);
  for (auto& b : p->yq) b.alloc(sizeof(Fr) * Q);
  p->slots.ensure(sizeof(MsmSlot) * ProofLayout{Q}.slots_total());
  p->prepared = true;
  API_END
}

void sonic_prover_free(sonic_prover_t* p) {
  if (!p) return;
  try { DeviceScope scope(p->device); delete p; } catch (const HipFail&) { delete p; }
}

size_t sonic_hsc_proof_size(int64_t m) { return (size_t)((2 + 4 * m) * 96 + (2 + 2 * m) * 32); }

int sonic_prover_hsc_prove(sonic_prover_t* p, int64_t m, const uint8_t* yzs, const uint8_t u[32], const uint8_t v[32], uint8_t* out) {
  API_BEGIN_ON(p ? p->device : -1)
  if (!p || m < 0 || (m > 0 && !yzs) || !u || !v || !out) return SONIC_ERR_INVALID_ARG;
  std::lock_guard<std::mutex> g(p->mu);
  if (p->in_flight) { set_error("sonic_prover_hsc_prove: a submitted proof has not been collected yet"); return SONIC_ERR_INVALID_ARG; }
  const long n = p->n, Q = p->Q, d = p->srs->d;
  for (long k = 0; k < 2 * m; k++)
    if (bytes_are_zero(yzs + 32 * k, 32)) { set_error("hscProve: y_j / z_j number %ld is zero: Laurent evaluation at 0 divides by zero", k); return SONIC_ERR_INEXACT_DIVISION; }
  if (bytes_are_zero(u, 32) || bytes_are_zero(v, 32)) { set_error("hscProve: u or v is zero"); return SONIC_ERR_INEXACT_DIVISION; }
  hipStream_t st = p->st;
  const sonic_srs* srs = p->srs;
  const long NS = 2 * m + 2;
  const long K = 4 * m + 2;
  DevBuf S(sizeof(Fr) * NS), PR(sizeof(Fr) * 2 * NS), slots(sizeof(MsmSlot) * K), frout(sizeof(Fr) * (2 * m + 1)), flags(4);
  DevBuf pw(sizeof(Fr) * (3 * n + Q + 2)), su(sizeof(Fr) * (2 * n + Q + 1)), sy(sizeof(Fr) * (3 * n + 1));
  int* fl = flags.as<int>();
  HIP_OK(hipMemsetAsync(fl, 0, 4, st));
  {
    std::vector<uint8_t> h(32 * (size_t)NS);
    for (long j = 0; j < m; j++) { memcpy(&h[32 * j], yzs + 64 * j, 32); memcpy(&h[32 * (m + j)], yzs + 64 * j + 32, 32); }
    memcpy(&h[32 * (2 * m)], u, 32); memcpy(&h[32 * (2 * m + 1)], v, 32);
    HIP_OK(hipMemcpyAsync(S.p, h.data(), h.size(), hipMemcpyHostToDevice, st));
    HIP_OK(hipStreamSynchronize(st));
  }
  fr_to_mont_enqueue(st, S.as<Fr>(), NS, fl);
  fr_with_inverse_enqueue(st, S.as<Fr>(), (int)NS, PR.as<Fr>());
  const Fr* P0 = PR.as<Fr>();
  auto pY = [&](long j) { return P0 + 2 * j; };
  auto pZ = [&](long j) { return P0 + 2 * (m + j); };
  const Fr *pU = P0 + 2 * (2 * m), *pV = P0 + 2 * (2 * m + 1);
  MsmSlot* sl = slots.as<MsmSlot>();
  Fr* fo = frout.as<Fr>();
  Lane& lane = p->lane_at(0);
  const long s_lo = -n, s_len = 3 * n + 1, u_lo = -n, u_len = 2 * n + Q + 1;
  for (long j = 0; j < m; j++) {
    poly_scale_powers_enqueue(st, nullptr, pw.as<Fr>(), 2 * n + Q + 1, -n, pY(j), pY(j) + 1);
    s_of_y_of(p, st, pw.as<Fr>(), sy.as<Fr>());
    MsmJob jobs[3];
    jobs[0] = commit_job(st, srs, sy.as<Fr>(), s_lo, s_len, d, &sl[3 * j], fl);
    jobs[1] = open_job(st, srs, lane.sc[1], sy.as<Fr>(), s_lo, s_len, pZ(j), &fo[j], &sl[3 * j + 1], fl);
    jobs[2] = open_job(st, srs, lane.sc[2], sy.as<Fr>(), s_lo, s_len, pU, nullptr, &sl[3 * j + 2], fl);
    run_jobs(st, srs, lane.ws, jobs, 3);
  }
  poly_scale_powers_enqueue(st, nullptr, pw.as<Fr>(), 3 * n + 1, -n, pU, pU + 1);
  s_of_u_of(p, st, pw.as<Fr>(), su.as<Fr>());
  {
    MsmJob jobs[MSM_MAX_JOBS];
    int k = 0;
    auto flush = [&] { run_jobs(st, srs, lane.ws, jobs, k); k = 0; };
    jobs[k++] = commit_job(st, srs, su.as<Fr>(), u_lo, u_len, d, &sl[4 * m + 1], fl);
    for (long j = 0; j < m; j++) {
      if (k == MSM_MAX_JOBS) flush();
      jobs[k] = open_job(st, srs, lane.sc[k], su.as<Fr>(), u_lo, u_len, pY(j), &fo[m + j], &sl[3 * m + j], fl);
      k++;
    }
    if (k == MSM_MAX_JOBS) flush();
    jobs[k] = open_job(st, srs, lane.sc[k], su.as<Fr>(), u_lo, u_len, pV, &fo[2 * m], &sl[4 * m], fl);
    k++;
    flush();
  }
  fr_from_mont_enqueue(st, fo, 2 * m + 1);
  std::vector<MsmSlot> hs((size_t)K);
  std::vector<uint8_t> hfr(32 * (size_t)(2 * m + 1));
  HIP_OK(hipMemcpyAsync(hs.data(), sl, sizeof(MsmSlot) * K, hipMemcpyDeviceToHost, st));
  HIP_OK(hipMemcpyAsync(hfr.data(), fo, hfr.size(), hipMemcpyDeviceToHost, st));
  int hflags = read_flags(st, flags);
  if (hflags) return flags_to_status(hflags, "hscProve");
  std::vector<uint8_t> pts(96 * (size_t)K);
  {
    std::vector<G1XYZZ> sums((size_t)K);
    finish_slots_host(hs.data(), K, sums.data(), 16);
    g1_canonical_bytes_host_batch(sums.data(), (int)K, pts.data());
  }
  uint8_t* o = out;
  auto putG = [&](long i) { memcpy(o, &pts[96 * (size_t)i], 96); o += 96; };
  auto putF = [&](const uint8_t* b) { memcpy(o, b, 32); o += 32; };
  for (long j = 0; j < m; j++) { putG(3 * j); putF(&hfr[32 * j]); putG(3 * j + 1); }
  for (long j = 0; j < m; j++) { putF(&hfr[32 * (m + j)]); putG(3 * j + 2); putG(3 * m + j); }
  putG(4 * m); putG(4 * m + 1); putF(u); putF(v);
  API_END
}

}
```

sonic_amd/csrc/prove_multi.hip:

```cpp
#include "prover.hpp"

namespace {
constexpr size_t ONE_SHOT_SHELLS = 4;
}
namespace sonic {
void drop_one_shot_of(const sonic_srs* s) {
  DeviceCtx& c = current_ctx();
  std::vector<OneShotShell*> gone;
  {
    std::lock_guard<std::mutex> g(c.one_shot_mu);
    for (size_t i = 0; i < c.one_shot.size();) {
      OneShotShell* sh = static_cast<OneShotShell*>(c.one_shot[i]);
      if (sh->srs == s) { gone.push_back(sh); c.one_shot.erase(c.one_shot.begin() + (long)i); } else i++;
    }
  }
  for (OneShotShell* sh : gone) { delete sh->p; delete sh; }
}
}
extern "C" {
int sonic_one_shot_trim(int device) {
  int freed = 0;
  try {
    int ndev = 0;
    if (sonic_device_count(&ndev) != SONIC_OK) return 0;
    for (int d = 0; d < ndev; d++) {
      if (device >= 0 && d != device) continue;
      DeviceScope scope(d);
      DeviceCtx& c = scope.ctx();
      std::vector<void*> gone;
      { std::lock_guard<std::mutex> g(c.one_shot_mu); gone.swap(c.one_shot); }
      for (void* v : gone) { OneShotShell* sh = static_cast<OneShotShell*>(v); delete sh->p; delete sh; freed++; }
    }
  } catch (const HipFail&) {}
  return freed;
}

}

static OneShotShell* take_shell(DeviceCtx& ctx, const sonic_srs* srs, long n, long Q) {
  std::lock_guard<std::mutex> g(ctx.one_shot_mu);
  for (size_t i = ctx.one_shot.size(); i-- > 0;) {
    OneShotShell* c = static_cast<OneShotShell*>(ctx.one_shot[i]);
    if (c->srs == srs && c->p->n == n && c->p->Q == Q) { ctx.one_shot.erase(ctx.one_shot.begin() + (long)i); return c; }
  }
  return nullptr;
}
static void park_shell(DeviceCtx& ctx, OneShotShell* sh) {
  OneShotShell* evict = nullptr;
  {
    std::lock_guard<std::mutex> g(ctx.one_shot_mu);
    if (ctx.one_shot.size() >= ONE_SHOT_SHELLS) { evict = static_cast<OneShotShell*>(ctx.one_shot.front()); ctx.one_shot.erase(ctx.one_shot.begin()); }
    ctx.one_shot.push_back(sh);
  }
  if (evict) { delete evict->p; delete evict; }
}

static int one_shot_prove(const char* who, const sonic_srs_t* srs, const CircuitView& c, const uint8_t* aL, const uint8_t* aR, const uint8_t* aO,
                          const uint8_t* transcript, uint8_t* out_proof) {
  API_BEGIN_ON(srs_device(srs))
  if (!srs || !c.cs || !aL || !aR || !aO || !transcript || !out_proof) { set_error("%s: bad argument (need n >= 1, Q >= 1)", who); return SONIC_ERR_INVALID_ARG; }
  int rc = prover_admits(who, srs, c);
  if (rc) return rc;
  DeviceCtx& ctx = current_ctx();
  OneShotShell* sh = take_shell(ctx, srs, c.n, c.Q);
  if (sh) prover_hand_over(sh->p, c);
  else {
    sonic_prover_t* p = nullptr;
    rc = prover_new_impl(srs, c, &p);
    if (rc) return rc;
    sh = new OneShotShell{srs, p};
  }
  rc = prove_with_statement(sh->p, aL, aR, aO, nullptr, transcript, out_proof);
  sh->p->pend = sonic_prover::PendingCircuit();
  park_shell(ctx, sh);
  return rc;
  API_END
}

extern "C" {

int sonic_prove(const sonic_srs_t* srs, int64_t n, int64_t Q, const uint8_t* wL, const uint8_t* wR, const uint8_t* wO,
                const uint8_t* cs, const uint8_t* aL, const uint8_t* aR, const uint8_t* aO, const uint8_t* transcript,
                uint8_t* out_proof) {
  return one_shot_prove("sonic_prove", srs, dense_view(n, Q, wL, wR, wO, cs), aL, aR, aO, transcript, out_proof);
}

int sonic_prove_csr(const sonic_srs_t* srs, int64_t n, int64_t Q, const int64_t* row_ptr, const int64_t* col, const uint8_t* val,
                    const uint8_t* cs, const uint8_t* aL, const uint8_t* aR, const uint8_t* aO, const uint8_t* transcript, uint8_t* out_proof) {
  return one_shot_prove("sonic_prove_csr", srs, csr_view(n, Q, row_ptr, col, val, cs), aL, aR, aO, transcript, out_proof);
}

int sonic_prove_many(const sonic_srs_t* const* srs, int n_srs, int64_t n, int64_t Q, const sonic_statement_t* statements, int64_t K,
                     uint8_t* out_proofs, int* out_status) {
  if (!srs || n_srs < 1 || n_srs > 512 || n < 1 || Q < 1 || K < 0 || (K > 0 && (!statements || !out_proofs))) return SONIC_ERR_INVALID_ARG;
  for (int i = 0; i < n_srs; i++) if (!srs[i]) return SONIC_ERR_INVALID_ARG;
  const size_t psz = sonic_proof_size(Q);
  const int T = 2 * n_srs;
  std::vector<int> status((size_t)K, SONIC_OK);
  std::vector<std::string> errs((size_t)T);
  auto body = [&](int t) {
    const sonic_srs_t* s = srs[t % n_srs];
    for (int64_t i = t; i < K; i += T) {
      int rc = SONIC_ERR_HIP;
      try {
        const sonic_statement_t& st = statements[i];
        rc = sonic_prove(s, n, Q, st.wL, st.wR, st.wO, st.cs, st.aL, st.aR, st.aO, st.transcript, out_proofs + psz * (size_t)i);
        if (rc && errs[(size_t)t].empty()) { char b[512]; sonic_last_error(b, sizeof b); errs[(size_t)t] = b; }
      } catch (...) { rc = SONIC_ERR_HIP; }
      status[(size_t)i] = rc;
    }
  };
  {
    ThreadGroup th;
    for (int t = 1; t < T && t < K; t++) th.emplace_back(body, t);
    body(0);
    for (auto& x : th) x.join();
  }
  if (out_status) for (int64_t i = 0; i < K; i++) out_status[i] = status[(size_t)i];
  for (int64_t i = 0; i < K; i++)
    if (status[(size_t)i]) {
      const int t = (int)(i % T);
      set_error("sonic_prove_many, statement %ld (device %d): %s", (long)i, srs_device(srs[t % n_srs]), errs[(size_t)t].c_str());
      return status[(size_t)i];
    }
  return SONIC_OK;
}

int sonic_prover_device(const sonic_prover_t* p) { return p ? p->device : -1; }

int sonic_prove_shared(sonic_prover_t* const* provers, int world, const uint8_t* transcript, uint8_t* out_proof) {
  if (!provers || world < 1 || world > 1024 || !transcript || !out_proof) return SONIC_ERR_INVALID_ARG;
  for (int r = 0; r < world; r++) {
    if (!provers[r]) return SONIC_ERR_INVALID_ARG;
    if (provers[r]->n != provers[0]->n || provers[r]->Q != provers[0]->Q) { set_error("sonic_prove_shared: handle %d proves another circuit shape (n, Q) than handle 0", r); return SONIC_ERR_INVALID_ARG; }
    for (int q = 0; q < r; q++) if (provers[q] == provers[r]) { set_error("sonic_prove_shared: handle %d appears twice (one handle runs one share at a time)", r); return SONIC_ERR_INVALID_ARG; }
  }
  if (world == 1) {
    if (provers[0]->share_world > 1) { int rc = sonic_prover_set_share(provers[0], 0, 1); if (rc) return rc; }
    return sonic_prover_prove(provers[0], transcript, out_proof);
  }
  const long Q = provers[0]->Q;
  const size_t ssz = sonic_proof_share_size(Q);
  std::vector<uint8_t> shares(ssz * (size_t)world);
  std::vector<int> rcs((size_t)world, SONIC_OK);
  std::vector<std::string> errs((size_t)world);
  auto body = [&](int r) {
    sonic_prover_t* p = provers[r];
    int rc = SONIC_OK;
    try {
      bool placed;
      { std::lock_guard<std::mutex> g(p->mu); placed = p->share_world == world && p->share_rank == r; }
      if (!placed) rc = sonic_prover_set_share(p, r, world);
      if (!rc) rc = sonic_prover_prove_share(p, transcript, &shares[ssz * (size_t)r]);
      if (rc) { char b[512]; sonic_last_error(b, sizeof b); errs[(size_t)r] = b; }
    } catch (...) { rc = SONIC_ERR_HIP; }
    rcs[(size_t)r] = rc;
  };
  {
    ThreadGroup th;
    for (int r = 1; r < world; r++) th.emplace_back(body, r);
    body(0);
    for (auto& t : th) t.join();
  }
  for (int r = 0; r < world; r++)
    if (rcs[(size_t)r]) { set_error("sonic_prove_shared, rank %d (device %d): %s", r, provers[r]->device, errs[(size_t)r].c_str()); return rcs[(size_t)r]; }
  return sonic_proof_from_shares(Q, world, shares.data(), transcript, out_proof);
}

struct BatchFs { const uint8_t *circuit_digests, *blinder_seeds; uint8_t* out_transcripts; };
static int prove_batch_impl(const char* who, sonic_prover_t* const* provers, int n_provers, int64_t K, const uint8_t* aL, const uint8_t* aR, const uint8_t* aO,
                            const uint8_t* cs, const uint8_t* transcripts, uint8_t* out_proofs, int* out_status, const BatchFs* fs = nullptr,
                            const sonic_witness_src_t* src = nullptr, bool from_src = false) {
  if (!provers || n_provers < 1 || n_provers > 1024 || K < 0 || (K > 0 && (!(fs ? fs->circuit_digests && fs->blinder_seeds : transcripts != nullptr) || !out_proofs))) return SONIC_ERR_INVALID_ARG;
  const bool per_proof = aL || aR || aO;
  if (per_proof && !(aL && aR && aO)) { set_error("%s: aL, aR, aO must be given together (or all NULL: the handles' resident assignments)", who); return SONIC_ERR_INVALID_ARG; }
  for (int i = 0; i < n_provers; i++) {
    if (!provers[i]) return SONIC_ERR_INVALID_ARG;
    if (provers[i]->n != provers[0]->n || provers[i]->Q != provers[0]->Q) { set_error("%s: handle %d proves another circuit shape (n, Q) than handle 0", who, i); return SONIC_ERR_INVALID_ARG; }
    if (provers[i]->share_world > 1) { set_error("%s: handle %d runs one rank's share of a proof (sonic_prover_set_share)", who, i); return SONIC_ERR_INVALID_ARG; }
    for (int q = 0; q < i; q++) if (provers[q] == provers[i]) { set_error("%s: handle %d appears twice", who, i); return SONIC_ERR_INVALID_ARG; }
  }
  const long n = provers[0]->n, Q = provers[0]->Q;
  WitnessView wv;
  WitnessReady ready;
  if (from_src && K > 0) {
    int rc = witness_view_of(who, src, n, K, &wv);
    if (rc) return rc;
    try {
      DeviceScope scope(provers[0]->device);
      for (int i = 0; i < n_provers && !rc; i++) rc = witness_on_device_of(who, wv, n, K, provers[i]->device);
      if (!rc) ready.record(wv);
    } catch (const HipFail& f) { return f.code; }
    if (rc) return rc;
  }
  const size_t psz = sonic_proof_size(Q), tsz = 32 * (size_t)(8 + 2 * Q), asz = 32 * (size_t)n, ksz = 32 * (size_t)Q;
  std::vector<int> status((size_t)K, SONIC_OK);
  std::vector<std::string> errs((size_t)n_provers);
  std::vector<int64_t> first_bad((size_t)n_provers, -1);
  auto body = [&](int h) {
    for (int64_t i = h; i < K; i += n_provers) {
      int rc = SONIC_OK;
      try {
        for (long q = 0; cs && q < Q && !rc; q++) {
          Fr k;
          memcpy(k.l, cs + ksz * (size_t)i + 32 * (size_t)q, 32);
          if (!fp_is_canonical(k)) { set_error("%s: cs[%ld] of proof %ld is not a canonical field element", who, q, (long)i); rc = SONIC_ERR_BAD_ENCODING; }
        }
        const uint8_t *aLi = per_proof ? aL + asz * (size_t)i : nullptr, *aRi = per_proof ? aR + asz * (size_t)i : nullptr, *aOi = per_proof ? aO + asz * (size_t)i : nullptr;
        const uint8_t* csi = cs ? cs + ksz * (size_t)i : nullptr;
        uint8_t* out = out_proofs + psz * (size_t)i;
        if (rc) {}
        else if (from_src && fs) rc = prove_fs_with_witness(provers[h], wv.block(i), ready.ev, csi, fs->circuit_digests + 32 * (size_t)i, fs->blinder_seeds + 32 * (size_t)i, out,
                                                            fs->out_transcripts ? fs->out_transcripts + tsz * (size_t)i : nullptr);
        else if (from_src) rc = prove_with_witness(provers[h], wv.block(i), ready.ev, csi, transcripts + tsz * (size_t)i, out);
        else if (fs) rc = prove_fs_with_statement(provers[h], aLi, aRi, aOi, csi, fs->circuit_digests + 32 * (size_t)i, fs->blinder_seeds + 32 * (size_t)i, out,
                                                  fs->out_transcripts ? fs->out_transcripts + tsz * (size_t)i : nullptr);
        else if (cs || per_proof) rc = prove_with_statement(provers[h], aLi, aRi, aOi, csi, transcripts + tsz * (size_t)i, out);
        else rc = sonic_prover_prove(provers[h], transcripts + tsz * (size_t)i, out);
        if (rc && first_bad[(size_t)h] < 0) { first_bad[(size_t)h] = i; char b[512]; sonic_last_error(b, sizeof b); errs[(size_t)h] = b; }
      } catch (...) { rc = SONIC_ERR_HIP; }
      status[(size_t)i] = rc;
    }
  };
  {
    ThreadGroup th;
    for (int h = 1; h < n_provers && h < K; h++) th.emplace_back(body, h);
    body(0);
    for (auto& t : th) t.join();
  }
  if (out_status) for (int64_t i = 0; i < K; i++) out_status[i] = status[(size_t)i];
  for (int64_t i = 0; i < K; i++)
    if (status[(size_t)i]) {
      const int h = (int)(i % n_provers);
      set_error("%s, proof %ld (handle %d, device %d): %s", who, (long)i, h, provers[h]->device, errs[(size_t)h].c_str());
      return status[(size_t)i];
    }
  return SONIC_OK;
}


int sonic_prove_batch(sonic_prover_t* const* provers, int n_provers, int64_t K, const uint8_t* aL, const uint8_t* aR, const uint8_t* aO,
                      const uint8_t* transcripts, uint8_t* out_proofs, int* out_status) {
  return prove_batch_impl("sonic_prove_batch", provers, n_provers, K, aL, aR, aO, nullptr, transcripts, out_proofs, out_status);
}

int sonic_prove_batch_statements(sonic_prover_t* const* provers, int n_provers, int64_t K, const uint8_t* aL, const uint8_t* aR, const uint8_t* aO,
                                 const uint8_t* cs, const uint8_t* transcripts, uint8_t* out_proofs, int* out_status) {
  try { DeviceScope probe(-1); } catch (const HipFail& f) { return f.code; }
  if (K > 0 && !cs) { set_error("sonic_prove_batch_statements: cs is NULL (sonic_prove_batch proves with the handles' constants)"); return SONIC_ERR_INVALID_ARG; }
  return prove_batch_impl("sonic_prove_batch_statements", provers, n_provers, K, aL, aR, aO, cs, transcripts, out_proofs, out_status);
}

int sonic_prove_batch_fs(sonic_prover_t* const* provers, int n_provers, int64_t K, const uint8_t* aL, const uint8_t* aR, const uint8_t* aO, const uint8_t* cs,
                         const uint8_t* circuit_digests, const uint8_t* blinder_seeds, uint8_t* out_proofs, uint8_t* out_transcripts, int* out_status) {
  try { DeviceScope probe(-1); } catch (const HipFail& f) { return f.code; }
  const BatchFs fs{circuit_digests, blinder_seeds, out_transcripts};
  return prove_batch_impl("sonic_prove_batch_fs", provers, n_provers, K, aL, aR, aO, cs, nullptr, out_proofs, out_status, &fs);
}

int sonic_prove_batch_src(sonic_prover_t* const* provers, int n_provers, int64_t K, const sonic_witness_src_t* src, const uint8_t* cs, const uint8_t* transcripts,
                          uint8_t* out_proofs, int* out_status) {
  try { DeviceScope probe(-1); } catch (const HipFail& f) { return f.code; }
  return prove_batch_impl("sonic_prove_batch_src", provers, n_provers, K, nullptr, nullptr, nullptr, cs, transcripts, out_proofs, out_status, nullptr, src, true);
}

int sonic_prove_batch_fs_src(sonic_prover_t* const* provers, int n_provers, int64_t K, const sonic_witness_src_t* src, const uint8_t* cs, const uint8_t* circuit_digests,
                             const uint8_t* blinder_seeds, uint8_t* out_proofs, uint8_t* out_transcripts, int* out_status) {
  try { DeviceScope probe(-1); } catch (const HipFail& f) { return f.code; }
  const BatchFs fs{circuit_digests, blinder_seeds, out_transcripts};
  return prove_batch_impl("sonic_prove_batch_fs_src", provers, n_provers, K, nullptr, nullptr, nullptr, cs, nullptr, out_proofs, out_status, &fs, src, true);
}

}
```

sonic_amd/csrc/prover.hpp:

```cpp
#pragma once
#include <string.h>
#include <algorithm>
#include <chrono>
#include <condition_variable>
#include <functional>
#include <memory>
#include <thread>
#include <numeric>
#include <string>
#include <vector>
#include "srs_handle.hpp"
#include "poly.hpp"
#include "fs.hpp"
#include "share_plan.hpp"
#include "csr.hpp"
#include "witness_src.hpp"


namespace sonic {


enum { FLAG_BAD_ENCODING = 1, FLAG_SRS_INDEX = 2 };
enum { PH_R = 1,
       PH_T = 2,
       PH_OPEN = 3,
       PH_HSCS = 4,
       PH_HSCW = 5,
       PH_QV = 6,
       PH_ALL = 0x7e };
constexpr int CQ_TAB_W = 29, CQ_TAB_C = 9;
constexpr long CQ_TAB_MAX_Q = 1L << 16;
struct Scratch {
  DevBuf D, q, scan, fz_discard;
  void reserve(long len) { D.ensure(sizeof(Fr) * (len + 1)); q.ensure(sizeof(Fr) * (len + 1)); fz_discard.ensure(sizeof(Fr)); }
};

MsmJob commit_job(hipStream_t st, const sonic_srs* srs, const Fr* poly, long lo, long len, long maxm, MsmSlot* slot, int* d_flags);
void run_jobs(hipStream_t st, const sonic_srs* srs, MsmWorkspace& ws, const MsmJob* jobs, int k, bool last = false, bool exposed = true);
MsmJob open_job(hipStream_t st, const sonic_srs* srs, Scratch& sc, const Fr* poly, long lo, long len,
                       const Fr* zpair, Fr* d_fz, MsmSlot* slot, int* d_flags);
MsmJob open_job_at_zero(hipStream_t st, const sonic_srs* srs, const Fr* poly, long len, Fr* d_fz, MsmSlot* slot, int* d_flags);
bool bytes_are_zero(const uint8_t* p, size_t n);

}

using namespace sonic;

struct Lane {
  hipStream_t st = nullptr;
  hipEvent_t done = nullptr;
  hipEvent_t prep = nullptr;
  MsmWorkspace ws;
  Scratch sc[MSM_MAX_JOBS];
  MsmJob jobs[MSM_MAX_JOBS];
  int njobs = 0;
};
constexpr int N_LANES = 6;

struct FsWorker {
  std::thread th;
  std::mutex m;
  std::condition_variable cv;
  bool has_job = false, done = false, quit = false;
  uint8_t circuit_digest[32], seed[32];
  int rc = 0;
  std::string err;
  std::vector<uint8_t> proof, transcript;
};

struct sonic_prover {
  const sonic_srs* srs = nullptr;
  int device = 0;
  long n = 0, Q = 0;
  hipStream_t st = nullptr;
  hipStream_t ts = nullptr;
  bool have_assignment = false;
  DevBuf wL, wR, wO, cs, aL, aR, aO;
  bool csr = false;
  struct CsrBufs {
    DevBuf row_ptr, col, val, col_ptr, row, cval, chunk_row, chunk_begin, row_chunk, partial;
    long nnz = 0, nchunks = 0;
    std::vector<int32_t> h_row_ptr;
  } sp;
  Lane lanes[N_LANES];
  int n_lanes = N_LANES;
  Lane chain[2];
  bool small_plan = false;
  int next_lane = 0;
  const NttTables* ntt = nullptr;
  DevBuf S, PAIRS, r1, sy0, su, pw, kpow, fa, fb, slots, frout, flags, tmp;
  std::vector<DevBuf> syj;
  uint8_t* h_tr = nullptr;
  Fr* h_pairs = nullptr;
  MsmSlot* h_slots = nullptr;
  uint8_t* h_fr = nullptr;
  int* h_flags = nullptr;
  struct PendingCircuit { bool set = false; CircuitView view = {}; CsrLayout layout; } pend;
  const uint8_t* pend_asg[3] = {nullptr, nullptr, nullptr};
  const uint8_t* pend_cs = nullptr;
  struct PendingWitness { bool set = false; WitnessView v; hipEvent_t ready = nullptr; } pend_wit;
  DevBuf wit_raw;
  struct StatementBufs { DevBuf stage, partial, out, gates; } stm;
  struct RunBufs {
    DevBuf masked, val, uniform, scal, pts;
    hipEvent_t masked_ev = nullptr;
  };
  MsmWorkspace runs_ws;
  std::vector<RunBufs> runs;
  bool runs_on = false;
  bool circuit_has_runs = true;
  bool sym_on = false;
  bool fused = false;
  std::vector<MsmJob> fused_jobs;
  std::vector<std::unique_ptr<Scratch>> fused_sc;
  size_t fused_sc_next = 0;
  Scratch& fused_scratch() {
    if (fused_sc_next == fused_sc.size()) fused_sc.emplace_back(new Scratch());
    return *fused_sc[fused_sc_next++];
  }
  bool use_graph = false;
  hipGraphExec_t graph = nullptr;
  bool graph_tried = false;
  long proofs_done = 0;
  bool in_flight = false;
  bool fs_flight = false;
  std::unique_ptr<FsWorker> fsw;
  uint32_t phases = 0x7e;
  DevBuf frstd;
  std::chrono::steady_clock::time_point t_begin, t_enq;
  bool prepared = false;
  DevBuf cq;
  DevBuf cq_tab;
  std::vector<DevBuf> diag, yq;
  hipEvent_t ev_r1 = nullptr, ev_sy0 = nullptr, ev_t = nullptr, ev_su = nullptr;
  std::vector<hipEvent_t> ev_syj;
  int log2m = 0;
  std::mutex mu;
  int share_rank = 0, share_world = 0;
  SharePlan share;
  bool share_planned_prepared = false, share_planned = false;
  int32_t share_plan_tag = 0;
  std::vector<uint8_t> slot_ran;
  std::vector<uint8_t> fr_valid;
  uint8_t witness_digest[32] = {0};
  bool have_witness_digest = false;
  uint8_t witness_digest_v2[32] = {0};
  bool have_witness_digest_v2 = false;
  DevBuf wtree;
  uint32_t* h_root = nullptr;
  void assignment_changed() { have_witness_digest = false; have_witness_digest_v2 = false; }
  Lane& lane_at(int i) { return lanes[i % n_lanes]; }
  Lane& pick(hipEvent_t ready) {
    Lane& l = lanes[next_lane];
    next_lane = (next_lane + 1) % (n_lanes > 1 ? n_lanes - 1 : 1);
    (void)hipStreamWaitEvent(l.st, ready, 0);
    return l;
  }
  Lane& t_lane(hipEvent_t ready) {
    Lane& l = lanes[n_lanes - 1];
    (void)hipStreamWaitEvent(l.st, ready, 0);
    return l;
  }
  ~sonic_prover() {
    if (fsw) {
      { std::lock_guard<std::mutex> g(fsw->m); fsw->quit = true; }
      fsw->cv.notify_all();
      if (fsw->th.joinable()) fsw->th.join();
    }
    for (auto& l : lanes) { if (l.st) (void)hipStreamDestroy(l.st); if (l.done) (void)hipEventDestroy(l.done); if (l.prep) (void)hipEventDestroy(l.prep); }
    for (auto& l : chain) { if (l.st) (void)hipStreamDestroy(l.st); if (l.done) (void)hipEventDestroy(l.done); if (l.prep) (void)hipEventDestroy(l.prep); }
    for (auto& r : runs) if (r.masked_ev) (void)hipEventDestroy(r.masked_ev);
    for (hipEvent_t e : {ev_r1, ev_sy0, ev_t, ev_su}) if (e) (void)hipEventDestroy(e);
    for (hipEvent_t e : ev_syj) if (e) (void)hipEventDestroy(e);
    if (st) (void)hipStreamDestroy(st);
    if (ts) (void)hipStreamDestroy(ts);
    if (graph) (void)hipGraphExecDestroy(graph);
    for (void* h : {(void*)h_tr, (void*)h_pairs, (void*)h_slots, (void*)h_fr, (void*)h_flags, (void*)h_root}) if (h) (void)hipHostFree(h);
  }
};

int upload_fr_mont(hipStream_t st, DevBuf& dst, const uint8_t* src, long count, int* d_flags);
int flags_to_status(int f, const char* who);
extern "C" int prove_with_statement(sonic_prover_t* p, const uint8_t* aL, const uint8_t* aR, const uint8_t* aO, const uint8_t* cs, const uint8_t* transcript,
                                    uint8_t* out_proof);
extern "C" int prove_fs_with_statement(sonic_prover_t* p, const uint8_t* aL, const uint8_t* aR, const uint8_t* aO, const uint8_t* cs, const uint8_t circuit_digest[32],
                                       const uint8_t blinder_seed[32], uint8_t* out_proof, uint8_t* out_transcript);
extern "C" int prove_with_witness(sonic_prover_t* p, const WitnessView& w, hipEvent_t ready, const uint8_t* cs, const uint8_t* transcript, uint8_t* out_proof);
extern "C" int prove_fs_with_witness(sonic_prover_t* p, const WitnessView& w, hipEvent_t ready, const uint8_t* cs, const uint8_t circuit_digest[32],
                                     const uint8_t blinder_seed[32], uint8_t* out_proof, uint8_t* out_transcript);
namespace sonic {
int witness_view_of(const char* who, const sonic_witness_src_t* src, long n, long B, WitnessView* out);
int witness_on_device_of(const char* who, const WitnessView& v, long n, long B, int device);
void witness_load_enqueue(sonic_prover* p, hipStream_t st, const WitnessView& v, long nb, Fr* oL, Fr* oR, Fr* oO, long out_stride, int* d_err);
struct WitnessReady {
  hipEvent_t ev = nullptr;
  WitnessReady() {}
  WitnessReady(const WitnessReady&) = delete;
  WitnessReady& operator=(const WitnessReady&) = delete;
  void record(const WitnessView& v);
  ~WitnessReady() { if (ev) (void)hipEventDestroy(ev); }
};
}
namespace sonic { const uint32_t* witness_tree_enqueue(hipStream_t st, const Fr* aL, const Fr* aR, const Fr* aO, long n, DevBuf& tree); }
int prover_admits(const char* who, const sonic_srs* srs, const CircuitView& c);
int prover_new_impl(const sonic_srs_t* srs, const CircuitView& c, sonic_prover_t** out);
void prover_hand_over(sonic_prover_t* p, const CircuitView& c);
```

sonic_amd/csrc/statement.hip:

```cpp
#include "prover.hpp"

namespace sonic {
namespace {

constexpr int CS_BLOCK = 256;
constexpr long STAGE_ELEMS = 1L << 20;
constexpr long PARTIAL_ELEMS = 1L << 20;

__device__ __forceinline__ Fr cs_shfl_xor(const Fr& a, int mask) {
  Fr o;
#pragma unroll
  for (int k = 0; k < 8; k++) o.l[k] = (uint32_t)__shfl_xor((int)a.l[k], mask, 64);
  return o;
}
__device__ __forceinline__ Fr cs_wave_sum(Fr acc) {
#pragma unroll
  for (int o = 32; o >= 1; o >>= 1) acc = fp_add(acc, cs_shfl_xor(acc, o));
  return acc;
}

__global__ __launch_bounds__(CS_BLOCK) void k_cs_csr(const int32_t* __restrict__ row_ptr, const int32_t* __restrict__ col, const Fr* __restrict__ val,
                                                     const int32_t* __restrict__ chunk_row, const int32_t* __restrict__ chunk_begin, long nchunks, int Q,
                                                     const Fr* __restrict__ aL, const Fr* __restrict__ aR, const Fr* __restrict__ aO, long stride,
                                                     Fr* __restrict__ partial) {
  const long c = (long)blockIdx.x * 4 + (threadIdx.x >> 6);
  const int lane = threadIdx.x & 63;
  if (c >= nchunks) return;
  const long b = blockIdx.y;
  const int r = chunk_row[c], m = r / Q;
  const int k0 = chunk_begin[c];
  const int k1 = min(k0 + CSR_CHUNK, row_ptr[r + 1]);
  const Fr* a = (m == 0 ? aL : m == 1 ? aR : aO) + b * stride;
  Fr acc = Fr::zero();
  for (int k = k0 + lane; k < k1; k += 64) acc = fp_add(acc, fp_mul(val[k], a[col[k]]));
  acc = cs_wave_sum(acc);
  if (lane == 0) partial[b * nchunks + c] = acc;
}

__global__ __launch_bounds__(CS_BLOCK) void k_cs_dense(const Fr* __restrict__ wL, const Fr* __restrict__ wR, const Fr* __restrict__ wO, long n, int Q,
                                                       const Fr* __restrict__ aL, const Fr* __restrict__ aR, const Fr* __restrict__ aO, long stride,
                                                       long nblk, Fr* __restrict__ partial) {
  __shared__ Fr sh[CS_BLOCK / 64];
  const long b = blockIdx.y, i = (long)blockIdx.x * CS_BLOCK + threadIdx.x;
  const bool in = i < n;
  Fr l = Fr::zero(), r = Fr::zero(), o = Fr::zero();
  if (in) { l = aL[b * stride + i]; r = aR[b * stride + i]; o = aO[b * stride + i]; }
  for (int q = 0; q < Q; q++) {
    Fr acc = Fr::zero();
    if (in) {
      const long at = (long)q * n + i;
      acc = fp_add(fp_add(fp_mul(wL[at], l), fp_mul(wR[at], r)), fp_mul(wO[at], o));
    }
    acc = cs_wave_sum(acc);
    if ((threadIdx.x & 63) == 0) sh[threadIdx.x >> 6] = acc;
    __syncthreads();
    if (threadIdx.x == 0) partial[(b * Q + q) * nblk + blockIdx.x] = fp_add(fp_add(sh[0], sh[1]), fp_add(sh[2], sh[3]));
    __syncthreads();
  }
}

__global__ __launch_bounds__(CS_BLOCK) void k_cs_finish(const int32_t* __restrict__ row_chunk, long per, int Q, const Fr* __restrict__ partial, Fr* __restrict__ out) {
  __shared__ Fr sh[CS_BLOCK];
  const int q = blockIdx.x;
  const long b = blockIdx.y;
  Fr acc = Fr::zero();
  if (row_chunk) {
    const Fr* p = partial + b * per;
    for (int m = 0; m < 3; m++) {
      const int r = m * Q + q;
      for (int c = row_chunk[r] + (int)threadIdx.x; c < row_chunk[r + 1]; c += CS_BLOCK) acc = fp_add(acc, p[c]);
    }
  } else {
    const Fr* p = partial + (b * Q + q) * per;
    for (long c = threadIdx.x; c < per; c += CS_BLOCK) acc = fp_add(acc, p[c]);
  }
  sh[threadIdx.x] = acc;
  __syncthreads();
  for (int s = CS_BLOCK / 2; s >= 1; s >>= 1) {
    if ((int)threadIdx.x < s) sh[threadIdx.x] = fp_add(sh[threadIdx.x], sh[threadIdx.x + s]);
    __syncthreads();
  }
  if (threadIdx.x == 0) out[b * Q + q] = fp_from_mont(sh[0]);
}

__global__ __launch_bounds__(CS_BLOCK) void k_gates(const Fr* __restrict__ aL, const Fr* __restrict__ aR, const Fr* __restrict__ aO, long stride, long n,
                                                    unsigned long long* __restrict__ gates) {
  __shared__ unsigned long long first[CS_BLOCK];
  __shared__ unsigned int count[CS_BLOCK];
  const long b = blockIdx.y, i = (long)blockIdx.x * CS_BLOCK + threadIdx.x;
  bool bad = false;
  if (i < n) bad = !(fp_mul(aL[b * stride + i], aR[b * stride + i]) == aO[b * stride + i]);
  first[threadIdx.x] = bad ? (unsigned long long)i : ~0ull;
  count[threadIdx.x] = bad ? 1u : 0u;
  __syncthreads();
  for (int s = CS_BLOCK / 2; s >= 1; s >>= 1) {
    if ((int)threadIdx.x < s) {
      count[threadIdx.x] += count[threadIdx.x + s];
      if (first[threadIdx.x + s] < first[threadIdx.x]) first[threadIdx.x] = first[threadIdx.x + s];
    }
    __syncthreads();
  }
  if (threadIdx.x == 0 && count[0]) {
    atomicAdd(&gates[2 * b], (unsigned long long)count[0]);
    atomicMin(&gates[2 * b + 1], first[0]);
  }
}

}
}

static int eval_constraints_run(const char* who, sonic_prover_t* p, int64_t B, const uint8_t* aL, const uint8_t* aR, const uint8_t* aO, const WitnessView* w,
                                uint8_t* out_cs, int64_t* out_gates) {
  const bool resident = !aL && !w;
  const long n = p->n, Q = p->Q;
  hipStream_t st = p->st;
  sonic_prover::CsrBufs& sp = p->sp;
  sonic_prover::StatementBufs& sb = p->stm;
  const long nblk = (n + CS_BLOCK - 1) / CS_BLOCK;
  const long per_b = p->csr ? sp.nchunks : Q * nblk;
  long Bc = std::min<long>(B, std::max<long>(1, STAGE_ELEMS / n));
  Bc = std::min<long>(Bc, std::max<long>(1, PARTIAL_ELEMS / std::max<long>(1, per_b)));
  Bc = std::min<long>(Bc, 65535);
  if (!resident) sb.stage.ensure(sizeof(Fr) * 3 * (size_t)Bc * (size_t)n);
  sb.partial.ensure(sizeof(Fr) * (size_t)Bc * (size_t)std::max<long>(1, per_b));
  sb.out.ensure(sizeof(Fr) * (size_t)Bc * (size_t)Q);
  sb.gates.ensure(16 * (size_t)Bc);
  std::vector<unsigned long long> gates_init(2 * (size_t)Bc), gates_host(2 * (size_t)Bc);
  for (long b = 0; b < Bc; b++) { gates_init[2 * (size_t)b] = 0; gates_init[2 * (size_t)b + 1] = ~0ull; }
  HIP_OK(hipMemsetAsync(p->flags.p, 0, 4, st));
  for (long b0 = 0; b0 < B; b0 += Bc) {
    const long nb = std::min<long>(Bc, B - b0);
    const Fr *dL = p->aL.as<Fr>(), *dR = p->aR.as<Fr>(), *dO = p->aO.as<Fr>();
    if (w) {
      Fr* s = sb.stage.as<Fr>();
      witness_load_enqueue(p, st, w->block(b0), nb, s, s + nb * n, s + 2 * nb * n, n, p->flags.as<int>());
      dL = s; dR = s + nb * n; dO = s + 2 * nb * n;
    } else if (!resident) {
      Fr* s = sb.stage.as<Fr>();
      const size_t bytes = 32 * (size_t)nb * (size_t)n, off = 32 * (size_t)b0 * (size_t)n;
      HIP_OK(hipMemcpyAsync(s, aL + off, bytes, hipMemcpyHostToDevice, st));
      HIP_OK(hipMemcpyAsync(s + nb * n, aR + off, bytes, hipMemcpyHostToDevice, st));
      HIP_OK(hipMemcpyAsync(s + 2 * nb * n, aO + off, bytes, hipMemcpyHostToDevice, st));
      fr_to_mont_enqueue(st, s, 3 * nb * n, p->flags.as<int>());
      dL = s; dR = s + nb * n; dO = s + 2 * nb * n;
    }
    Fr* partial = sb.partial.as<Fr>();
    if (p->csr) {
      if (sp.nchunks > 0)
        LAUNCH(k_cs_csr, dim3((unsigned)ceil_div(sp.nchunks, 4L), (unsigned)nb), CS_BLOCK, 0, st, (const int32_t*)sp.row_ptr.as<int32_t>(), (const int32_t*)sp.col.as<int32_t>(),
               (const Fr*)sp.val.as<Fr>(), (const int32_t*)sp.chunk_row.as<int32_t>(), (const int32_t*)sp.chunk_begin.as<int32_t>(), sp.nchunks, (int)Q, dL, dR, dO, n, partial);
      LAUNCH(k_cs_finish, dim3((unsigned)Q, (unsigned)nb), CS_BLOCK, 0, st, (const int32_t*)sp.row_chunk.as<int32_t>(), sp.nchunks, (int)Q, (const Fr*)partial, sb.out.as<Fr>());
    } else {
      LAUNCH(k_cs_dense, dim3((unsigned)nblk, (unsigned)nb), CS_BLOCK, 0, st, (const Fr*)p->wL.as<Fr>(), (const Fr*)p->wR.as<Fr>(), (const Fr*)p->wO.as<Fr>(), n, (int)Q, dL, dR, dO, n,
             nblk, partial);
      LAUNCH(k_cs_finish, dim3((unsigned)Q, (unsigned)nb), CS_BLOCK, 0, st, (const int32_t*)nullptr, nblk, (int)Q, (const Fr*)partial, sb.out.as<Fr>());
    }
    HIP_OK(hipMemcpyAsync(out_cs + 32 * (size_t)b0 * (size_t)Q, sb.out.p, 32 * (size_t)nb * (size_t)Q, hipMemcpyDeviceToHost, st));
    const bool gates_derived = w && !w->aO;
    if (out_gates && !gates_derived) {
      HIP_OK(hipMemcpyAsync(sb.gates.p, gates_init.data(), 16 * (size_t)nb, hipMemcpyHostToDevice, st));
      LAUNCH(k_gates, dim3((unsigned)nblk, (unsigned)nb), CS_BLOCK, 0, st, dL, dR, dO, n, n, sb.gates.as<unsigned long long>());
      HIP_OK(hipMemcpyAsync(gates_host.data(), sb.gates.p, 16 * (size_t)nb, hipMemcpyDeviceToHost, st));
    }
    HIP_OK(hipStreamSynchronize(st));
    for (long b = 0; out_gates && gates_derived && b < nb; b++) { out_gates[2 * (b0 + b)] = 0; out_gates[2 * (b0 + b) + 1] = -1; }
    for (long b = 0; out_gates && !gates_derived && b < nb; b++) {
      out_gates[2 * (b0 + b)] = (int64_t)gates_host[2 * (size_t)b];
      out_gates[2 * (b0 + b) + 1] = gates_host[2 * (size_t)b] ? (int64_t)gates_host[2 * (size_t)b + 1] : -1;
    }
  }
  const int f = read_flags(st, p->flags);
  if (f) return flags_to_status(f, who);
  return SONIC_OK;
}

extern "C" {

int sonic_prover_eval_constraints(sonic_prover_t* p, int64_t B, const uint8_t* aL, const uint8_t* aR, const uint8_t* aO, uint8_t* out_cs, int64_t* out_gates) {
  API_BEGIN_ON(p ? p->device : -1)
  const char* who = "sonic_prover_eval_constraints";
  if (!p || !out_cs) { set_error("%s: bad argument", who); return SONIC_ERR_INVALID_ARG; }
  const bool resident = !aL && !aR && !aO;
  if (!resident && !(aL && aR && aO)) { set_error("%s: aL, aR, aO must be given together (or all NULL: the handle's resident assignment)", who); return SONIC_ERR_INVALID_ARG; }
  const long n = p->n;
  if (B < 1 || B > MSM_TABLE_MAX_TERMS / n) { set_error("%s: B = %lld outside [1, 2^26 / n]", who, (long long)B); return SONIC_ERR_INVALID_ARG; }
  if (resident && B != 1) { set_error("%s: the resident assignment is one assignment (B = 1)", who); return SONIC_ERR_INVALID_ARG; }
  std::lock_guard<std::mutex> g(p->mu);
  if (resident && !p->have_assignment) { set_error("%s: no assignment set", who); return SONIC_ERR_INVALID_ARG; }
  if (p->in_flight) { set_error("%s: a submitted proof is still reading the handle's buffers (collect it first)", who); return SONIC_ERR_INVALID_ARG; }
  return eval_constraints_run(who, p, B, aL, aR, aO, nullptr, out_cs, out_gates);
  API_CATCH
}

int sonic_prover_eval_constraints_src(sonic_prover_t* p, int64_t B, const sonic_witness_src_t* src, uint8_t* out_cs, int64_t* out_gates) {
  API_BEGIN_ON(p ? p->device : -1)
  const char* who = "sonic_prover_eval_constraints_src";
  if (!p || !out_cs) { set_error("%s: bad argument", who); return SONIC_ERR_INVALID_ARG; }
  const long n = p->n;
  if (B < 1 || B > MSM_TABLE_MAX_TERMS / n) { set_error("%s: B = %lld outside [1, 2^26 / n]", who, (long long)B); return SONIC_ERR_INVALID_ARG; }
  WitnessView v;
  int rc = witness_view_of(who, src, n, B, &v);
  if (rc) return rc;
  std::lock_guard<std::mutex> g(p->mu);
  if (p->in_flight) { set_error("%s: a submitted proof is still reading the handle's buffers (collect it first)", who); return SONIC_ERR_INVALID_ARG; }
  rc = witness_on_device_of(who, v, n, B, p->device);
  if (rc) return rc;
  WitnessReady ready;
  ready.record(v);
  if (ready.ev) HIP_OK(hipStreamWaitEvent(p->st, ready.ev, 0));
  return eval_constraints_run(who, p, B, nullptr, nullptr, nullptr, &v, out_cs, out_gates);
  API_CATCH
}

int sonic_prover_set_constants(sonic_prover_t* p, const uint8_t* cs) {
  API_BEGIN_ON(p ? p->device : -1)
  if (!p || !cs) { set_error("sonic_prover_set_constants: bad argument"); return SONIC_ERR_INVALID_ARG; }
  std::lock_guard<std::mutex> g(p->mu);
  if (p->in_flight) { set_error("sonic_prover_set_constants: a submitted proof is still reading the current constants (collect it first)"); return SONIC_ERR_INVALID_ARG; }
  for (long q = 0; q < p->Q; q++) {
    Fr k;
    memcpy(k.l, cs + 32 * q, 32);
    if (!fp_is_canonical(k)) { set_error("sonic_prover_set_constants: cs[%ld] is not a canonical field element", q); return SONIC_ERR_BAD_ENCODING; }
  }
  HIP_OK(hipMemsetAsync(p->flags.p, 0, 4, p->st));
  upload_fr_mont(p->st, p->cs, cs, p->Q, p->flags.as<int>());
  HIP_OK(hipStreamSynchronize(p->st));
  API_END
}

int sonic_fs_circuit_midstate(int64_t n, int64_t Q, const uint8_t* wL, const uint8_t* wR, const uint8_t* wO, uint8_t out[SONIC_FS_MIDSTATE_SIZE]) {
  return circuit_midstate_checked("sonic_fs_circuit_midstate", dense_view(n, Q, wL, wR, wO, nullptr), out);
}
int sonic_fs_circuit_midstate_csr(int64_t n, int64_t Q, const int64_t* row_ptr, const int64_t* col, const uint8_t* val, uint8_t out[SONIC_FS_MIDSTATE_SIZE]) {
  return circuit_midstate_checked("sonic_fs_circuit_midstate_csr", csr_view(n, Q, row_ptr, col, val, nullptr), out);
}
int sonic_fs_circuit_digest_resume(const uint8_t midstate[SONIC_FS_MIDSTATE_SIZE], const uint8_t* cs, uint8_t out[32]) {
  if (!midstate || !cs || !out) { set_error("sonic_fs_circuit_digest_resume: bad argument"); return SONIC_ERR_INVALID_ARG; }
  int64_t bad = -1;
  const int rc = fs_circuit_digest_resume(midstate, cs, out, &bad);
  if (rc == 1) { set_error("sonic_fs_circuit_digest_resume: the midstate's length field is not 36 + 96 Q n for its Q (or bytes follow the pending ones)"); return SONIC_ERR_INVALID_ARG; }
  if (rc == 2) { set_error("sonic_fs_circuit_digest_resume: cs[%lld] is not a canonical field element", (long long)bad); return SONIC_ERR_BAD_ENCODING; }
  return SONIC_OK;
}
int sonic_verify_batch_digest_v2(int64_t n, int64_t Q, int64_t d, const uint8_t circuit_digest[32], const uint8_t srs_id[32], int64_t K, const uint8_t* proofs,
                                 const uint8_t* challenges, const uint8_t* cs, uint8_t out[32]) {
  if (n < 1 || Q < 1 || d < 1 || K < 0 || !circuit_digest || !srs_id || !out || (K > 0 && (!proofs || !challenges || !cs))) { set_error("sonic_verify_batch_digest_v2: bad argument"); return SONIC_ERR_INVALID_ARG; }
  fs_batch_digest_v2(n, Q, d, circuit_digest, srs_id, K, proofs, sonic_proof_size(Q), challenges, cs, out);
  return SONIC_OK;
}

}
```

sonic_amd/csrc/witness_src.hip:

```cpp
#include "prover.hpp"

namespace sonic {
namespace {

constexpr int WI_BLOCK = 256;

template <int KIND>
__device__ __forceinline__ bool wit_load(const uint8_t* __restrict__ v, long i, Fr& out) {
  if constexpr (KIND == SONIC_WIT_I64) {
    out = wit_i64_to_fr(*reinterpret_cast<const int64_t*>(v + 8 * i));
    return true;
  } else {
    const uint4* q = reinterpret_cast<const uint4*>(v + 32 * i);
    const uint4 lo = q[0], hi = q[1];
    out.l[0] = lo.x; out.l[1] = lo.y; out.l[2] = lo.z; out.l[3] = lo.w;
    out.l[4] = hi.x; out.l[5] = hi.y; out.l[6] = hi.z; out.l[7] = hi.w;
    return fp_is_canonical(out);
  }
}
__device__ __forceinline__ void wit_store(Fr* __restrict__ plane, long at, const Fr& v) {
  uint4* o = reinterpret_cast<uint4*>(plane + at);
  o[0] = make_uint4(v.l[0], v.l[1], v.l[2], v.l[3]);
  o[1] = make_uint4(v.l[4], v.l[5], v.l[6], v.l[7]);
}

template <int KIND, bool HAS_AO>
__global__ __launch_bounds__(WI_BLOCK) void k_witness_ingest(const uint8_t* __restrict__ aL, const uint8_t* __restrict__ aR, const uint8_t* __restrict__ aO, long stride, long n,
                                                             Fr* __restrict__ oL, Fr* __restrict__ oR, Fr* __restrict__ oO, long out_stride, int* __restrict__ err) {
  const long i = (long)blockIdx.x * WI_BLOCK + threadIdx.x, b = blockIdx.y;
  if (i >= n) return;
  Fr l, r, o = Fr::zero();
  bool ok = wit_load<KIND>(aL + b * stride, i, l);
  ok = wit_load<KIND>(aR + b * stride, i, r) && ok;
  if constexpr (HAS_AO) ok = wit_load<KIND>(aO + b * stride, i, o) && ok;
  if (ok) {
    l = fp_to_mont(l);
    r = fp_to_mont(r);
    if constexpr (HAS_AO) o = fp_to_mont(o);
    else o = fp_mul(l, r);
  } else {
    atomicOr(err, FLAG_BAD_ENCODING);
    l = r = o = Fr::zero();
  }
  const long at = b * out_stride + i;
  wit_store(oL, at, l);
  wit_store(oR, at, r);
  wit_store(oO, at, o);
}

void witness_ingest_enqueue(hipStream_t st, const WitnessView& v, long nb, long n, Fr* oL, Fr* oR, Fr* oO, long out_stride, int* d_err) {
  const dim3 grid((unsigned)ceil_div(n, WI_BLOCK), (unsigned)nb);
  const bool i64 = v.kind == SONIC_WIT_I64;
  if (i64 && v.aO) LAUNCH((k_witness_ingest<SONIC_WIT_I64, true>), grid, WI_BLOCK, 0, st, v.aL, v.aR, v.aO, (long)v.stride, n, oL, oR, oO, out_stride, d_err);
  else if (i64) LAUNCH((k_witness_ingest<SONIC_WIT_I64, false>), grid, WI_BLOCK, 0, st, v.aL, v.aR, v.aO, (long)v.stride, n, oL, oR, oO, out_stride, d_err);
  else if (v.aO) LAUNCH((k_witness_ingest<SONIC_WIT_FR32, true>), grid, WI_BLOCK, 0, st, v.aL, v.aR, v.aO, (long)v.stride, n, oL, oR, oO, out_stride, d_err);
  else LAUNCH((k_witness_ingest<SONIC_WIT_FR32, false>), grid, WI_BLOCK, 0, st, v.aL, v.aR, v.aO, (long)v.stride, n, oL, oR, oO, out_stride, d_err);
}

}

int witness_view_of(const char* who, const sonic_witness_src_t* src, long n, long B, WitnessView* out) {
  char msg[256];
  const int rc = wit_view_checked(src, n, B, out, msg, sizeof msg);
  if (rc) set_error("%s: %s", who, msg);
  return rc;
}

int witness_on_device_of(const char* who, const WitnessView& v, long n, long B, int device) {
  if (!v.on_device) return SONIC_OK;
  const uint8_t* ptr[3] = {v.aL, v.aR, v.aO};
  const char* name[3] = {"aL", "aR", "aO"};
  const size_t need = (size_t)(B - 1) * (size_t)v.stride + (size_t)n * (size_t)v.elem();
  for (int k = 0; k < 3; k++) {
    if (!ptr[k]) continue;
    hipPointerAttribute_t at;
    const hipError_t e = hipPointerGetAttributes(&at, ptr[k]);
    if (e != hipSuccess || at.type == hipMemoryTypeUnregistered || at.type == hipMemoryTypeHost) {
      if (e != hipSuccess) (void)hipGetLastError();
      set_error("%s: on_device = 1, but %s is a host pointer, not memory of device %d (the handle's GPU)", who, name[k], device);
      return SONIC_ERR_INVALID_ARG;
    }
    if (at.type != hipMemoryTypeDevice) { set_error("%s: %s is neither host nor plain device memory (memory type %d); the handle lives on device %d", who, name[k], (int)at.type, device); return SONIC_ERR_INVALID_ARG; }
    if (at.device != device) {
      set_error("%s: %s lies on device %d, the handle on device %d (a device source must lie on the GPU of every handle that reads it; no peer copy is made)", who, name[k], at.device, device);
      return SONIC_ERR_INVALID_ARG;
    }
    hipDeviceptr_t base = nullptr;
    size_t size = 0;
    if (hipMemGetAddressRange(&base, &size, (hipDeviceptr_t)ptr[k]) != hipSuccess) { (void)hipGetLastError(); continue; }
    const size_t off = (size_t)(ptr[k] - static_cast<const uint8_t*>(base));
    if (off > size || need > size - off) {
      set_error("%s: %s needs %zu bytes (%ld assignments of %ld elements), its allocation has %zu from there", who, name[k], need, B, n, size - (off > size ? size : off));
      return SONIC_ERR_INVALID_ARG;
    }
  }
  return SONIC_OK;
}

void WitnessReady::record(const WitnessView& v) {
  if (!v.on_device || !v.hip_stream) return;
  if (!ev) HIP_OK(hipEventCreateWithFlags(&ev, hipEventDisableTiming));
  HIP_OK(hipEventRecord(ev, static_cast<hipStream_t>(v.hip_stream)));
}

void witness_load_enqueue(sonic_prover* p, hipStream_t st, const WitnessView& v, long nb, Fr* oL, Fr* oR, Fr* oO, long out_stride, int* d_err) {
  const long n = p->n;
  WitnessView d = v;
  if (!v.on_device) {
    const size_t row = (size_t)n * (size_t)v.elem(), plane = (size_t)nb * row;
    const uint8_t* src[3] = {v.aL, v.aR, v.aO};
    p->wit_raw.ensure((v.aO ? 3 : 2) * plane);
    uint8_t* raw = p->wit_raw.as<uint8_t>();
    for (int k = 0; k < 3; k++) {
      if (!src[k]) continue;
      if ((size_t)v.stride == row) HIP_OK(hipMemcpyAsync(raw + k * plane, src[k], plane, hipMemcpyHostToDevice, st));
      else for (long b = 0; b < nb; b++) HIP_OK(hipMemcpyAsync(raw + k * plane + (size_t)b * row, src[k] + (size_t)b * (size_t)v.stride, row, hipMemcpyHostToDevice, st));
    }
    d.aL = raw; d.aR = raw + plane; d.aO = v.aO ? raw + 2 * plane : nullptr;
    d.stride = (int64_t)row; d.on_device = true;
  }
  witness_ingest_enqueue(st, d, nb, n, oL, oR, oO, out_stride, d_err);
}

}

extern "C" {

int sonic_prover_set_witness(sonic_prover_t* p, const sonic_witness_src_t* src) {
  API_BEGIN_ON(p ? p->device : -1)
  const char* who = "sonic_prover_set_witness";
  if (!p) { set_error("%s: bad argument", who); return SONIC_ERR_INVALID_ARG; }
  WitnessView v;
  int rc = witness_view_of(who, src, p->n, 1, &v);
  if (rc) return rc;
  std::lock_guard<std::mutex> g(p->mu);
  if (p->in_flight) { set_error("%s: a submitted proof is still reading the current assignment (collect it first)", who); return SONIC_ERR_INVALID_ARG; }
  rc = witness_on_device_of(who, v, p->n, 1, p->device);
  if (rc) return rc;
  WitnessReady ready;
  ready.record(v);
  hipStream_t st = p->st;
  for (DevBuf* b : {&p->aL, &p->aR, &p->aO}) b->ensure(sizeof(Fr) * (size_t)p->n);
  if (ready.ev) HIP_OK(hipStreamWaitEvent(st, ready.ev, 0));
  HIP_OK(hipMemsetAsync(p->flags.p, 0, 4, st));
  p->have_assignment = false;
  p->assignment_changed();
  witness_load_enqueue(p, st, v, 1, p->aL.as<Fr>(), p->aR.as<Fr>(), p->aO.as<Fr>(), p->n, p->flags.as<int>());
  const int f = read_flags(st, p->flags);
  if (f) return flags_to_status(f, who);
  p->have_assignment = true;
  API_END
}

}
```

Baseline: 29.76 proofs/s.

## Map prover streams onto a shared per-device pool sized to hardware queues

Adds a per-device pool of prover streams, sized from GPU_MAX_HW_QUEUES or SONIC_STREAM_POOL, and maps roles onto it: head, NTT, MSM lanes, chains and a tail stream for the final copies. It also stops forcing GPU_MAX_HW_QUEUES to 8, and stages assignment uploads on a separate upload stream ordered by an event. The aim is to avoid streams oversubscribing the hardware queues and the false serialization that can cause, and to let uploads overlap with other work. In exchange, handles now share streams, so a device-wide enqueue mutex and extra event joins are needed, and lanes that share a pooled stream may lose concurrency.

```diff
diff --git a/sonic_amd/csrc/device.hip b/sonic_amd/csrc/device.hip
--- a/sonic_amd/csrc/device.hip
+++ b/sonic_amd/csrc/device.hip
@@ -40,7 +40,6 @@
 
 static int device_count_locked() {
   if (g_device_count >= 0) return g_device_count;
-  setenv("GPU_MAX_HW_QUEUES", "8", 0);
   int n = 0;
   hipError_t e = hipGetDeviceCount(&n);
   if (e != hipSuccess || n <= 0) {
@@ -111,6 +110,17 @@
   }
   return *t;
 }
+int device_prover_streams() {
+  DeviceCtx& c = current_ctx();
+  std::lock_guard<std::mutex> g(c.pool_mu);
+  if (c.prover_streams < 0) {
+    const int n = pool_size_of_env(getenv("GPU_MAX_HW_QUEUES"), getenv("SONIC_STREAM_POOL"));
+    if (n > 0) c.prover_stream[0] = c.stream;
+    for (int i = 1; i < n; i++) HIP_OK(hipStreamCreateWithFlags(&c.prover_stream[i], hipStreamNonBlocking));
+    c.prover_streams = n;
+  }
+  return c.prover_streams;
+}
 DeviceCtx& current_ctx() {
   if (!t_ctx) { set_error("internal: no device scope on this thread"); throw HipFail{SONIC_ERR_HIP}; }
   return *t_ctx;
diff --git a/sonic_amd/csrc/internal.hpp b/sonic_amd/csrc/internal.hpp
--- a/sonic_amd/csrc/internal.hpp
+++ b/sonic_amd/csrc/internal.hpp
@@ -4,6 +4,7 @@
 #include "common.hpp"
 #include "g1.hpp"
 #include "msm.hpp"
+#include "stream_pool.hpp"
 
 struct sonic_srs;
 struct sonic_prover;
@@ -16,6 +17,9 @@
 struct DeviceCtx {
   int dev = -1;
   hipStream_t stream = nullptr;
+  int prover_streams = -1;
+  hipStream_t prover_stream[POOL_MAX] = {};
+  std::mutex enqueue_mu;
   std::mutex call_mu;
   std::mutex pool_mu;
   std::vector<CallCtx*> pool;
@@ -47,6 +51,11 @@
 DeviceCtx& current_ctx();
 int default_device_ordinal();
 inline hipStream_t default_stream() { return current_ctx().stream; }
+int device_prover_streams();
+inline hipStream_t device_prover_stream(PoolRole role, int k = 0) {
+  DeviceCtx& c = current_ctx();
+  return c.prover_stream[pool_stream_of(role, k, c.prover_streams)];
+}
 inline std::mutex& call_mutex() { return current_ctx().call_mu; }
 struct CallCtx { hipStream_t st = nullptr; MsmWorkspace ws; };
 class CallLease {
diff --git a/sonic_amd/csrc/prove.hip b/sonic_amd/csrc/prove.hip
--- a/sonic_amd/csrc/prove.hip
+++ b/sonic_amd/csrc/prove.hip
@@ -4,6 +4,7 @@
 namespace sonic {
 
 constexpr long PROVE_TWO_LEVEL_MAX_TERMS = 1L << 21;
+constexpr long POOL_MAX_TERMS = 1L << 21;
 static bool prove_two_level(const MsmPlan& pl, int k, bool last, long nmax) {
   if (last || k <= 1 || pl.NB < (1 << 18)) return false;
   const char* e = getenv("SONIC_PROVE_TWO_LEVEL");
@@ -223,7 +224,7 @@
   return circuit_validate(who, c);
 }
 
-int prover_new_impl(const sonic_srs_t* srs, const CircuitView& c, sonic_prover_t** out) {
+int prover_new_impl(const sonic_srs_t* srs, const CircuitView& c, sonic_prover_t** out, bool own_streams) {
   const long n = c.n, Q = c.Q;
   const ProofLayout L{Q};
   for (long q = 0; c.csr && q < Q; q++) {
@@ -237,10 +238,18 @@
     const MsmPlan probe = srs_msm_plan(srs, 3 * n);
     p->small_plan = msm_can_batch(probe) && probe.NB <= (1 << 17);
   }
-  auto mkstream = [](hipStream_t* s) { HIP_OK(hipStreamCreateWithFlags(s, hipStreamNonBlocking)); };
-  mkstream(&p->st);
-  mkstream(&p->ts);
+  p->use_graph = getenv("SONIC_PROVE_GRAPH") && atoi(getenv("SONIC_PROVE_GRAPH")) != 0;
+  const bool pool_size_ok = 7 * n + 9 <= POOL_MAX_TERMS || (getenv("SONIC_STREAM_POOL") && atoi(getenv("SONIC_STREAM_POOL")) > 0);
+  p->pooled = !p->use_graph && !own_streams && pool_size_ok && device_prover_streams() > 0;
+  auto mkstream = [&p](hipStream_t* s, PoolRole role, int k = 0) {
+    if (p->pooled) *s = device_prover_stream(role, k);
+    else HIP_OK(hipStreamCreateWithFlags(s, hipStreamNonBlocking));
+  };
+  mkstream(&p->st, PoolRole::HEAD);
+  mkstream(&p->ts, PoolRole::NTT);
+  p->tail = p->pooled ? device_prover_stream(PoolRole::TAIL) : p->st;
   hipStream_t st = p->st;
+  EnqueueLock enq(p.get());
   p->flags.alloc(8);
   int rc_c = prover_load_circuit(p.get(), c);
   if (rc_c) return rc_c;
@@ -260,7 +269,6 @@
   p->kpow.alloc(sizeof(Fr) * Q);
   p->S.alloc(sizeof(Fr) * L.transcript_len()); p->PAIRS.alloc(sizeof(Fr) * 2 * L.n_pairs());
   p->slots.alloc(sizeof(MsmSlot) * L.slots_total());
-  p->use_graph = getenv("SONIC_PROVE_GRAPH") && atoi(getenv("SONIC_PROVE_GRAPH")) != 0;
   HIP_OK(hipHostMalloc((void**)&p->h_tr, 32 * L.transcript_len(), hipHostMallocDefault));
   HIP_OK(hipHostMalloc((void**)&p->h_pairs, sizeof(Fr) * 2 * L.n_pairs(), hipHostMallocDefault));
   HIP_OK(hipHostMalloc((void**)&p->h_slots, sizeof(MsmSlot) * L.slots_total(), hipHostMallocDefault));
@@ -277,19 +285,21 @@
   mkev(&p->ev_r1); mkev(&p->ev_sy0); mkev(&p->ev_t); mkev(&p->ev_su);
   p->ev_syj.resize(Q, nullptr);
   for (auto& e : p->ev_syj) mkev(&e);
+  mkev(&p->done); mkev(&p->ev_head); mkev(&p->ev_ts);
   if (p->small_plan) {
     const char* le = getenv("SONIC_FUSED_LANES");
     p->n_lanes = std::min(std::max(le ? atoi(le) : N_LANES, 1), N_LANES);
   }
   for (int i = 0; i < p->n_lanes; i++) {
     Lane& l = p->lanes[i];
-    mkstream(&l.st);
+    const bool t_lane = i == p->n_lanes - 1;
+    if (t_lane && !p->small_plan) mkstream(&l.st, PoolRole::T_GROUP); else mkstream(&l.st, PoolRole::GROUP, t_lane ? i + 1 : i);
     mkev(&l.done);
     mkev(&l.prep);
   }
   if (p->small_plan) {
     for (int c = 0; c < (L.K() > MSM_MAX_JOBS ? 2 : 1); c++) {
-      mkstream(&p->chain[c].st);
+      mkstream(&p->chain[c].st, PoolRole::CHAIN, c);
       mkev(&p->chain[c].done);
     }
   }
@@ -306,6 +316,7 @@
   std::lock_guard<std::mutex> g(p->mu);
   if (p->in_flight) { set_error("sonic_prover_set_assignment: a submitted proof is still reading the current assignment (collect it first)"); return SONIC_ERR_INVALID_ARG; }
   hipStream_t st = p->st;
+  EnqueueLock enq(p);
   HIP_OK(hipMemsetAsync(p->flags.p, 0, 4, st));
   upload_fr_mont(st, p->aL, aL, p->n, p->flags.as<int>());
   upload_fr_mont(st, p->aR, aR, p->n, p->flags.as<int>());
@@ -458,7 +469,11 @@
     deferred_small.clear();
   }
   void join() {
-    hipStream_t ms = p->st;
+    hipStream_t ms = p->tail;
+    if (p->pooled) {
+      HIP_OK(hipEventRecord(p->ev_head, p->st)); HIP_OK(hipStreamWaitEvent(ms, p->ev_head, 0));
+      HIP_OK(hipEventRecord(p->ev_ts, p->ts)); HIP_OK(hipStreamWaitEvent(ms, p->ev_ts, 0));
+    }
     for (int i = 0; i < p->n_lanes; i++) { Lane& l = p->lanes[i]; HIP_OK(hipEventRecord(l.done, l.st)); HIP_OK(hipStreamWaitEvent(ms, l.done, 0)); }
     if (p->fused) for (auto& l : p->chain) if (l.st) { HIP_OK(hipEventRecord(l.done, l.st)); HIP_OK(hipStreamWaitEvent(ms, l.done, 0)); }
   }
@@ -622,11 +637,31 @@
   q.drain_deferred();
 }
 
+static void stage_assignment(sonic_prover_t* p) {
+  if (!p->up) {
+    HIP_OK(hipStreamCreateWithFlags(&p->up, hipStreamNonBlocking));
+    HIP_OK(hipEventCreateWithFlags(&p->ev_up, hipEventDisableTiming));
+  }
+  int* flags = p->flags.as<int>();
+  HIP_OK(hipMemsetAsync(flags + 1, 0, 4, p->up));
+  upload_fr_mont(p->up, p->aL, p->pend_asg[0], p->n, flags + 1);
+  upload_fr_mont(p->up, p->aR, p->pend_asg[1], p->n, flags + 1);
+  upload_fr_mont(p->up, p->aO, p->pend_asg[2], p->n, flags + 1);
+  HIP_OK(hipEventRecord(p->ev_up, p->up));
+  p->pend_asg[0] = nullptr;
+  p->assignment_changed();
+  p->asg_staged = true;
+}
+
 static void enqueue_proof(sonic_prover_t* p) {
   const ProofLayout L{p->Q};
   hipStream_t st = p->st;
   int* flags = p->flags.as<int>();
-  HIP_OK(hipMemsetAsync(flags, 0, 8, st));
+  if (p->asg_staged) {
+    HIP_OK(hipMemsetAsync(flags, 0, 4, st));
+    HIP_OK(hipStreamWaitEvent(st, p->ev_up, 0));
+    p->asg_staged = false;
+  } else HIP_OK(hipMemsetAsync(flags, 0, 8, st));
   Fr* S = p->S.as<Fr>();
   HIP_OK(hipMemcpyAsync(S, p->h_tr, 32 * L.transcript_len(), hipMemcpyHostToDevice, st));
   fr_to_mont_enqueue(st, S, L.transcript_len(), flags);
@@ -636,13 +671,15 @@
   enqueue_polynomials(p, q, w);
   enqueue_groups(p, q, w);
   q.join();
+  hipStream_t tl = p->tail;
   Fr* frstd = p->frstd.as<Fr>();
-  HIP_OK(hipMemcpyAsync(frstd, q.frout, sizeof(Fr) * L.F(), hipMemcpyDeviceToDevice, st));
-  fr_from_mont_enqueue(st, frstd, L.F());
+  HIP_OK(hipMemcpyAsync(frstd, q.frout, sizeof(Fr) * L.F(), hipMemcpyDeviceToDevice, tl));
+  fr_from_mont_enqueue(tl, frstd, L.F());
   const long KS = p->sym_on ? L.slots_total() : (p->prepared || p->runs_on) ? L.C_extra() : L.K();
-  HIP_OK(hipMemcpyAsync(p->h_slots, q.slots, sizeof(MsmSlot) * KS, hipMemcpyDeviceToHost, st));
-  HIP_OK(hipMemcpyAsync(p->h_fr, frstd, 32 * L.F(), hipMemcpyDeviceToHost, st));
-  HIP_OK(hipMemcpyAsync(p->h_flags, flags, 8, hipMemcpyDeviceToHost, st));
+  HIP_OK(hipMemcpyAsync(p->h_slots, q.slots, sizeof(MsmSlot) * KS, hipMemcpyDeviceToHost, tl));
+  HIP_OK(hipMemcpyAsync(p->h_fr, frstd, 32 * L.F(), hipMemcpyDeviceToHost, tl));
+  HIP_OK(hipMemcpyAsync(p->h_flags, flags, 8, hipMemcpyDeviceToHost, tl));
+  if (p->pooled) HIP_OK(hipEventRecord(p->done, tl));
 }
 
 static void decide_modes(sonic_prover_t* p) {
@@ -721,7 +758,8 @@
     ~CaptureGuard() { if (active) { hipGraph_t g = nullptr; (void)hipStreamEndCapture(st, &g); if (g) (void)hipGraphDestroy(g); } }
   } capture{st};
   if (capturing) { p->graph_tried = true; HIP_OK(hipStreamBeginCapture(st, hipStreamCaptureModeRelaxed)); capture.active = true; }
-  if (!replay) enqueue_proof(p);
+  if (p->pooled && p->pend_asg[0]) stage_assignment(p);
+  if (!replay) { EnqueueLock enq(p); enqueue_proof(p); }
   if (capturing) {
     hipGraph_t g = nullptr;
     capture.active = false;
@@ -747,7 +785,7 @@
 }
 
 static bool await_proof(sonic_prover_t* p, bool share) {
-  HIP_OK(hipStreamSynchronize(p->st));
+  p->await_done();
   p->proofs_done++;
   if (!getenv("SONIC_DEBUG_TIMING")) return false;
   char who[32] = "prove";
@@ -907,7 +945,17 @@
 
 static int prove_run(sonic_prover_t* p, const uint8_t* transcript, int (*finish)(sonic_prover_t*, uint8_t*), uint8_t* out) {
   int rc = prove_enqueue(p, transcript);
-  if (rc) { if (p->st) (void)hipStreamSynchronize(p->st); return rc; }
+  if (rc) {
+    if (p->st) (void)hipStreamSynchronize(p->st);
+    if (p->pooled) {
+      (void)hipStreamSynchronize(p->ts); (void)hipStreamSynchronize(p->tail);
+      if (p->up) (void)hipStreamSynchronize(p->up);
+      p->asg_staged = false;
+      for (auto& l : p->lanes) if (l.st) (void)hipStreamSynchronize(l.st);
+      for (auto& l : p->chain) if (l.st) (void)hipStreamSynchronize(l.st);
+    }
+    return rc;
+  }
   return finish ? finish(p, out) : SONIC_OK;
 }
 
@@ -979,6 +1027,7 @@
   p->share_rank = world > 1 ? rank : 0;
   p->share_world = world > 1 ? world : 0;
   p->share_planned = false;
+  EnqueueLock enq(p);
   HIP_OK(hipMemsetAsync(p->slots.p, 0, sizeof(MsmSlot) * ProofLayout{p->Q}.C_extra(), p->st));
   HIP_OK(hipMemsetAsync(p->frout.p, 0, sizeof(Fr) * ProofLayout{p->Q}.F(), p->st));
   HIP_OK(hipStreamSynchronize(p->st));
@@ -1027,6 +1076,7 @@
 static void witness_digest_v1_ensure(sonic_prover_t* p) {
   if (p->have_witness_digest) return;
   const long n = p->n;
+  EnqueueLock enq(p);
   DevBuf tmp(sizeof(Fr) * 3 * n);
   Fr* t3 = tmp.as<Fr>();
   HIP_OK(hipMemcpyAsync(t3, p->aL.p, sizeof(Fr) * n, hipMemcpyDeviceToDevice, p->st));
@@ -1057,6 +1107,7 @@
 }
 static void witness_digest_v2_ensure(sonic_prover_t* p) {
   if (p->have_witness_digest_v2) return;
+  EnqueueLock enq(p);
   witness_digest_v2_enqueue(p);
   HIP_OK(hipStreamSynchronize(p->st));
   witness_digest_v2_finish(p);
@@ -1206,6 +1257,7 @@
   if (!aL && !p->have_assignment) { set_error("prove: no assignment set"); return SONIC_ERR_INVALID_ARG; }
   hipStream_t st = p->st;
   if (aL) {
+    EnqueueLock enq(p);
     p->have_assignment = false;
     p->assignment_changed();
     HIP_OK(hipMemsetAsync(p->flags.p, 0, 4, st));
@@ -1236,12 +1288,15 @@
   p->have_assignment = false;
   p->assignment_changed();
   for (DevBuf* a : {&p->aL, &p->aR, &p->aO}) a->ensure(sizeof(Fr) * (size_t)p->n);
-  if (ready) HIP_OK(hipStreamWaitEvent(st, ready, 0));
-  HIP_OK(hipMemsetAsync(p->flags.p, 0, 4, st));
-  witness_load_enqueue(p, st, w, 1, p->aL.as<Fr>(), p->aR.as<Fr>(), p->aO.as<Fr>(), p->n, p->flags.as<int>());
-  witness_digest_v2_enqueue(p);
-  const int f = read_flags(st, p->flags);
-  if (f) return flags_to_status(f, "prove (assignment handed over with the call)");
+  {
+    EnqueueLock enq(p);
+    if (ready) HIP_OK(hipStreamWaitEvent(st, ready, 0));
+    HIP_OK(hipMemsetAsync(p->flags.p, 0, 4, st));
+    witness_load_enqueue(p, st, w, 1, p->aL.as<Fr>(), p->aR.as<Fr>(), p->aO.as<Fr>(), p->n, p->flags.as<int>());
+    witness_digest_v2_enqueue(p);
+    const int f = read_flags(st, p->flags);
+    if (f) return flags_to_status(f, "prove (assignment handed over with the call)");
+  }
   witness_digest_v2_finish(p);
   p->have_assignment = true;
   p->pend_cs = cs;
@@ -1261,6 +1316,7 @@
   p->graph_tried = false;
   const long n = p->n, Q = p->Q, d = p->srs->d;
   int* flags = p->flags.as<int>();
+  EnqueueLock enq(p);
   HIP_OK(hipMemsetAsync(flags, 0, 4, p->st));
   HIP_OK(hipStreamSynchronize(p->st));
   DevBuf slots(sizeof(MsmSlot) * Q);
@@ -1355,6 +1411,7 @@
     if (bytes_are_zero(yzs + 32 * k, 32)) { set_error("hscProve: y_j / z_j number %ld is zero: Laurent evaluation at 0 divides by zero", k); return SONIC_ERR_INEXACT_DIVISION; }
   if (bytes_are_zero(u, 32) || bytes_are_zero(v, 32)) { set_error("hscProve: u or v is zero"); return SONIC_ERR_INEXACT_DIVISION; }
   hipStream_t st = p->st;
+  EnqueueLock enq(p);
   const sonic_srs* srs = p->srs;
   const long NS = 2 * m + 2;
   const long K = 4 * m + 2;
diff --git a/sonic_amd/csrc/prove_multi.hip b/sonic_amd/csrc/prove_multi.hip
--- a/sonic_amd/csrc/prove_multi.hip
+++ b/sonic_amd/csrc/prove_multi.hip
@@ -66,7 +66,7 @@
   if (sh) prover_hand_over(sh->p, c);
   else {
     sonic_prover_t* p = nullptr;
-    rc = prover_new_impl(srs, c, &p);
+    rc = prover_new_impl(srs, c, &p, true);
     if (rc) return rc;
     sh = new OneShotShell{srs, p};
   }
diff --git a/sonic_amd/csrc/prover.hpp b/sonic_amd/csrc/prover.hpp
--- a/sonic_amd/csrc/prover.hpp
+++ b/sonic_amd/csrc/prover.hpp
@@ -74,6 +74,14 @@
   long n = 0, Q = 0;
   hipStream_t st = nullptr;
   hipStream_t ts = nullptr;
+  bool pooled = false;
+  hipStream_t tail = nullptr;
+  hipEvent_t done = nullptr;
+  hipEvent_t ev_head = nullptr, ev_ts = nullptr;
+  hipStream_t up = nullptr;
+  hipEvent_t ev_up = nullptr;
+  bool asg_staged = false;
+  void await_done() { if (pooled) HIP_OK(hipEventSynchronize(done)); else HIP_OK(hipStreamSynchronize(st)); }
   bool have_assignment = false;
   DevBuf wL, wR, wO, cs, aL, aR, aO;
   bool csr = false;
@@ -167,16 +175,29 @@
       fsw->cv.notify_all();
       if (fsw->th.joinable()) fsw->th.join();
     }
-    for (auto& l : lanes) { if (l.st) (void)hipStreamDestroy(l.st); if (l.done) (void)hipEventDestroy(l.done); if (l.prep) (void)hipEventDestroy(l.prep); }
-    for (auto& l : chain) { if (l.st) (void)hipStreamDestroy(l.st); if (l.done) (void)hipEventDestroy(l.done); if (l.prep) (void)hipEventDestroy(l.prep); }
+    if (pooled) {
+      if (done) (void)hipEventSynchronize(done);
+      for (auto& l : lanes) if (l.done) (void)hipEventSynchronize(l.done);
+      for (auto& l : chain) if (l.done) (void)hipEventSynchronize(l.done);
+      for (hipEvent_t e : {ev_head, ev_ts, ev_up}) if (e) (void)hipEventSynchronize(e);
+    }
+    if (up) (void)hipStreamDestroy(up);
+    if (ev_up) (void)hipEventDestroy(ev_up);
+    for (auto& l : lanes) { if (l.st && !pooled) (void)hipStreamDestroy(l.st); if (l.done) (void)hipEventDestroy(l.done); if (l.prep) (void)hipEventDestroy(l.prep); }
+    for (auto& l : chain) { if (l.st && !pooled) (void)hipStreamDestroy(l.st); if (l.done) (void)hipEventDestroy(l.done); if (l.prep) (void)hipEventDestroy(l.prep); }
     for (auto& r : runs) if (r.masked_ev) (void)hipEventDestroy(r.masked_ev);
-    for (hipEvent_t e : {ev_r1, ev_sy0, ev_t, ev_su}) if (e) (void)hipEventDestroy(e);
+    for (hipEvent_t e : {ev_r1, ev_sy0, ev_t, ev_su, done, ev_head, ev_ts}) if (e) (void)hipEventDestroy(e);
     for (hipEvent_t e : ev_syj) if (e) (void)hipEventDestroy(e);
-    if (st) (void)hipStreamDestroy(st);
-    if (ts) (void)hipStreamDestroy(ts);
+    if (st && !pooled) (void)hipStreamDestroy(st);
+    if (ts && !pooled) (void)hipStreamDestroy(ts);
     if (graph) (void)hipGraphExecDestroy(graph);
     for (void* h : {(void*)h_tr, (void*)h_pairs, (void*)h_slots, (void*)h_fr, (void*)h_flags, (void*)h_root}) if (h) (void)hipHostFree(h);
   }
+};
+
+struct EnqueueLock {
+  std::unique_lock<std::mutex> l;
+  explicit EnqueueLock(const sonic_prover* p) { if (p->pooled) l = std::unique_lock<std::mutex>(current_ctx().enqueue_mu); }
 };
 
 int upload_fr_mont(hipStream_t st, DevBuf& dst, const uint8_t* src, long count, int* d_flags);
@@ -203,5 +224,5 @@
 }
 namespace sonic { const uint32_t* witness_tree_enqueue(hipStream_t st, const Fr* aL, const Fr* aR, const Fr* aO, long n, DevBuf& tree); }
 int prover_admits(const char* who, const sonic_srs* srs, const CircuitView& c);
-int prover_new_impl(const sonic_srs_t* srs, const CircuitView& c, sonic_prover_t** out);
+int prover_new_impl(const sonic_srs_t* srs, const CircuitView& c, sonic_prover_t** out, bool own_streams = false);
 void prover_hand_over(sonic_prover_t* p, const CircuitView& c);
diff --git a/sonic_amd/csrc/statement.hip b/sonic_amd/csrc/statement.hip
--- a/sonic_amd/csrc/statement.hip
+++ b/sonic_amd/csrc/statement.hip
@@ -188,6 +188,7 @@
   std::lock_guard<std::mutex> g(p->mu);
   if (resident && !p->have_assignment) { set_error("%s: no assignment set", who); return SONIC_ERR_INVALID_ARG; }
   if (p->in_flight) { set_error("%s: a submitted proof is still reading the handle's buffers (collect it first)", who); return SONIC_ERR_INVALID_ARG; }
+  EnqueueLock enq(p);
   return eval_constraints_run(who, p, B, aL, aR, aO, nullptr, out_cs, out_gates);
   API_CATCH
 }
@@ -207,6 +208,7 @@
   if (rc) return rc;
   WitnessReady ready;
   ready.record(v);
+  EnqueueLock enq(p);
   if (ready.ev) HIP_OK(hipStreamWaitEvent(p->st, ready.ev, 0));
   return eval_constraints_run(who, p, B, nullptr, nullptr, nullptr, &v, out_cs, out_gates);
   API_CATCH
@@ -222,6 +224,7 @@
     memcpy(k.l, cs + 32 * q, 32);
     if (!fp_is_canonical(k)) { set_error("sonic_prover_set_constants: cs[%ld] is not a canonical field element", q); return SONIC_ERR_BAD_ENCODING; }
   }
+  EnqueueLock enq(p);
   HIP_OK(hipMemsetAsync(p->flags.p, 0, 4, p->st));
   upload_fr_mont(p->st, p->cs, cs, p->Q, p->flags.as<int>());
   HIP_OK(hipStreamSynchronize(p->st));
diff --git a/sonic_amd/csrc/stream_pool.hpp b/sonic_amd/csrc/stream_pool.hpp
--- /dev/null
+++ b/sonic_amd/csrc/stream_pool.hpp
@@ -0,0 +1,49 @@
+#pragma once
+#include <stdlib.h>
+
+namespace sonic {
+
+constexpr int POOL_MIN = 2, POOL_MAX = 32;
+constexpr int POOL_CAP = 8;
+constexpr int POOL_DEFAULT_QUEUES = 4;
+constexpr bool POOL_DEFAULT_ON = true;
+
+enum class PoolRole { HEAD, NTT, GROUP, T_GROUP, CHAIN, TAIL };
+
+inline int pool_stream_of(PoolRole role, int k, int P) {
+  if (P < POOL_MIN) P = POOL_MIN;
+  if (k < 0) k = 0;
+  if (P == 2) return role == PoolRole::HEAD || role == PoolRole::NTT ? 0 : 1;
+  const bool ntt_alone = P >= 5, chain_alone = P >= 6;
+  const int first = ntt_alone ? 2 : 1, cnt = P - 1 - first - (chain_alone ? 1 : 0);
+  switch (role) {
+    case PoolRole::HEAD: return 0;
+    case PoolRole::NTT: return 1;
+    case PoolRole::TAIL:
+    case PoolRole::T_GROUP: return P - 1;
+    case PoolRole::CHAIN: return chain_alone ? P - 2 : P - 1;
+    case PoolRole::GROUP: return first + (k + (ntt_alone ? 0 : 1)) % cnt;
+  }
+  return 0;
+}
+
+inline int pool_queues_of_env(const char* v) {
+  if (!v || !*v) return POOL_DEFAULT_QUEUES;
+  char* end = nullptr;
+  const long q = strtol(v, &end, 10);
+  if (end == v || *end) return POOL_DEFAULT_QUEUES;
+  return q < POOL_MIN ? POOL_MIN : q > POOL_MAX ? POOL_MAX : (int)q;
+}
+
+inline int pool_size_of_env(const char* queues, const char* knob, bool default_on = POOL_DEFAULT_ON) {
+  const int q = pool_queues_of_env(queues);
+  const int by_queues = q < POOL_CAP ? q : POOL_CAP;
+  if (knob && *knob) {
+    char* end = nullptr;
+    const long k = strtol(knob, &end, 10);
+    if (end != knob && !*end) return k <= 0 ? 0 : k < POOL_MIN ? POOL_MIN : k > POOL_MAX ? POOL_MAX : (int)k;
+  }
+  return default_on ? by_queues : 0;
+}
+
+}
diff --git a/sonic_amd/csrc/witness_src.hip b/sonic_amd/csrc/witness_src.hip
--- a/sonic_amd/csrc/witness_src.hip
+++ b/sonic_amd/csrc/witness_src.hip
@@ -141,6 +141,7 @@
   ready.record(v);
   hipStream_t st = p->st;
   for (DevBuf* b : {&p->aL, &p->aR, &p->aO}) b->ensure(sizeof(Fr) * (size_t)p->n);
+  EnqueueLock enq(p);
   if (ready.ev) HIP_OK(hipStreamWaitEvent(st, ready.ev, 0));
   HIP_OK(hipMemsetAsync(p->flags.p, 0, 4, st));
   p->have_assignment = false;
```

Measured after the change: 31.19 proofs/s, median of 6. 4.8% higher.
